# gerbenvoshol/kmer-cnt

Hardware: AMD Instinct MI355X
Metric: Mbases/sec (+ k-mers/sec) on 150 bp FASTQ, k=21 (higher is better)
Workload: dtype u8

## Files before the change

### include/vafc.h

```cpp
#ifndef VAFC_H
#define VAFC_H

#include <stddef.h>
#include <stdint.h>

#ifdef __cplusplus
extern "C" {
#endif

#define VAFC_VERSION_MAJOR 0
#define VAFC_VERSION_MINOR 1

enum {
	VC_OK = 0,
	VC_EINVAL = -1,
	VC_ENOMEM = -2,
	VC_EHIP = -3,
	VC_ENODEV = -4,
	VC_EIO = -5,
	VC_ETOOMANY = -6,
	VC_EFULL = -7
};

typedef struct vc_ctx vc_ctx;
typedef struct vc_patterns vc_patterns;


int vc_patterns_load(const char *path, vc_patterns **out);
void vc_patterns_free(vc_patterns *db);
int vc_patterns_count(const vc_patterns *db);

int vc_patterns_keys(const vc_patterns *db, int k, uint64_t **keys, uint32_t **vals,
                     size_t *n_keys, int *n_collisions);

int vc_write_vaf(const vc_patterns *db, const uint32_t *counts, const char *path);

int vc_pattern_fields(const vc_patterns *db, int i, const char **chr, int *start,
                      const char **rsid, char *ref, char *alt,
                      const char **ref_kmer, const char **alt_kmer);

void vc_free(void *p);


int vc_create(vc_ctx **out, int k, const uint64_t *keys, const uint32_t *vals,
              size_t n_keys, uint32_t n_patterns, int device);
void vc_destroy(vc_ctx *ctx);

int vc_count_block(vc_ctx *ctx, const uint8_t *seq, size_t seq_bytes,
                   const uint64_t *offs, const uint32_t *lens, uint64_t n_reads);

#define VC_STREAM_CTX ((void *)(intptr_t)-1)

int vc_count_device(vc_ctx *ctx, const uint8_t *d_seq, size_t seq_bytes,
                    const uint64_t *d_offs, const uint32_t *d_lens, uint64_t n_reads,
                    void *stream);

int vc_finish(vc_ctx *ctx, uint32_t *counts, uint64_t *kmers_extracted);

int vc_reset(vc_ctx *ctx);

void *vc_device_counts(vc_ctx *ctx);
int vc_bind_outputs(vc_ctx *ctx, void *d_counts, void *d_tally);
void *vc_device_tally(vc_ctx *ctx);
void *vc_stream(vc_ctx *ctx);

int vc_set_timing(vc_ctx *ctx, int enable);
int vc_kernel_ms(vc_ctx *ctx, float *ms);

int vc_table_info(const vc_ctx *ctx, uint64_t *n_keys, uint64_t *slots, uint64_t *filter_bytes);


#define VC_MAX_SHARDS 64

int vc_create_multi(vc_ctx **out, int k, const uint64_t *keys, const uint32_t *vals, size_t n_keys,
                    uint32_t n_patterns, const int *devices, int n_devices);
int vc_shard_count(const vc_ctx *ctx);
int vc_shard_info(const vc_ctx *ctx, int i, int *device, uint64_t *batches);


typedef struct {
	uint64_t bases;
	uint64_t seqs;
	uint64_t blocks;
	double seconds;
} vc_file_stats;

int vc_count_file(vc_ctx *ctx, const char *path, int block_bases, int n_threads,
                  vc_file_stats *st);

typedef struct {
	uint64_t first;
	uint64_t next;
	uint64_t errs;
	uint32_t stopped;
	uint32_t whole;
} vc_range_info;
int vc_count_file_range(vc_ctx *ctx, const char *path, uint64_t begin, uint64_t end, int block_bases,
                        int n_threads, vc_file_stats *st, vc_range_info *ri);
int vc_scan_file_range(const char *path, int k, int block_bases, int n_threads, uint64_t piece_bytes,
                       uint64_t begin, uint64_t end, vc_file_stats *st, vc_range_info *ri, uint8_t *seq_out,
                       size_t seq_cap, uint32_t *lens_out, size_t lens_cap);

uint64_t vc_ingest_profile(double *prof);

#define VC_INGEST_PROFILE_FIELDS 17
uint64_t vc_ingest_profile_ex(double *prof, int n);

int vc_reserve_file_ingest(vc_ctx *ctx, int n_threads);

int vc_scan_file(const char *path, int k, int block_bases, vc_file_stats *st,
                 uint8_t *seq_out, size_t seq_cap, uint32_t *lens_out, size_t lens_cap);

int vc_scan_file_parallel(const char *path, int k, int block_bases, int n_threads, uint64_t piece_bytes,
                          vc_file_stats *st, uint8_t *seq_out, size_t seq_cap, uint32_t *lens_out,
                          size_t lens_cap);

int64_t vc_gz_inflate_parallel(const char *path, int n_threads, uint64_t chunk_bytes, uint8_t *out,
                               uint64_t cap, uint64_t *stats6);
int64_t vc_gz_inflate_zlib(const char *path, uint8_t *out, uint64_t cap);
uint32_t vc_gz_crc32(uint32_t crc, const uint8_t *p, uint64_t n);
uint32_t vc_gz_crc32_combine(uint32_t crc1, uint32_t crc2, uint64_t len2);

typedef struct {
	uint64_t start_bit;
	uint64_t end_bit;
	uint64_t text_len;
	uint32_t ok;
	uint32_t ended;
} vc_gz_share_info;
int vc_gz_share_scan(const char *path, uint64_t begin, uint64_t end, int n_threads, uint64_t chunk_bytes,
                     vc_gz_share_info *out, uint16_t *window_sym);

typedef struct {
	uint32_t events;
	uint32_t head_crc;
	uint64_t head_len;
	uint32_t head_expect_crc;
	uint32_t head_expect_isize;
	uint32_t tail_crc;
	uint64_t tail_len;
	uint32_t crc_error;
	uint32_t complete;
} vc_gz_share_crc;
int vc_count_gz_share(vc_ctx *ctx, const char *path, int first_share, uint64_t start_bit, const uint8_t *window,
                      uint64_t text_len, int block_bases, int n_threads, vc_file_stats *st, vc_range_info *ri,
                      vc_gz_share_crc *crc);
int vc_scan_gz_share(const char *path, int k, int first_share, uint64_t start_bit, const uint8_t *window,
                     uint64_t text_len, int block_bases, int n_threads, vc_file_stats *st, vc_range_info *ri,
                     vc_gz_share_crc *crc, uint8_t *seq_out, size_t seq_cap, uint32_t *lens_out, size_t lens_cap);

typedef struct vc_gz_share vc_gz_share;
int vc_gz_share_open(vc_ctx *ctx, const char *path, uint64_t begin, uint64_t end, int n_threads,
                     uint64_t chunk_bytes, uint64_t hold_bytes, vc_gz_share_info *out, uint16_t *window_sym,
                     vc_gz_share **held);
int vc_count_gz_share_held(vc_ctx *ctx, vc_gz_share *held, int first_share, const uint8_t *window, uint64_t text_len,
                           int block_bases, int n_threads, vc_file_stats *st, vc_range_info *ri, vc_gz_share_crc *crc);
int vc_scan_gz_share_held(vc_gz_share *held, int k, int first_share, const uint8_t *window, uint64_t text_len,
                          int block_bases, int n_threads, vc_file_stats *st, vc_range_info *ri, vc_gz_share_crc *crc,
                          uint8_t *seq_out, size_t seq_cap, uint32_t *lens_out, size_t lens_cap);
void vc_gz_share_close(vc_gz_share *held);

int64_t vc_scan_records(const char *path, int32_t *rets, int64_t cap);


typedef struct vc_fasta vc_fasta;
int vc_fasta_load(const char *path, vc_fasta **out);
int vc_fasta_count(const vc_fasta *fa);
const char *vc_fasta_name(const vc_fasta *fa, int i);
const uint8_t *vc_fasta_seq(const vc_fasta *fa, int i, uint32_t *len);
int vc_fasta_data(const vc_fasta *fa, const uint8_t **seq, size_t *bytes, const uint64_t **offs,
                  const uint32_t **lens);
void vc_fasta_free(vc_fasta *fa);


int vc_kc_create(vc_ctx **out, int k, uint64_t table_slots, int device);
int vc_kc_set_partition(vc_ctx *ctx, uint32_t n_parts, uint32_t part);
uint64_t vc_kc_slots(vc_ctx *ctx);
int vc_kc_histogram(vc_ctx *ctx, uint64_t *hist, uint64_t *distinct, uint64_t *kmers);
int vc_kc_histogram2(vc_ctx *ctx, uint64_t *hist, uint32_t n_bins, uint64_t min_count, uint64_t *distinct,
                     uint64_t *kmers);

int vc_kc_track_first(vc_ctx *ctx, int on);
int vc_yak_bloom_select(vc_ctx *ctx, int pre, int bf_shift, int n_hash);

int vc_set_nt4_decode(vc_ctx *ctx, int on);

int vc_count_candidates(int k, const uint8_t *seq, size_t seq_bytes, const uint64_t *offs,
                        const uint32_t *lens, uint64_t n_seqs, const uint64_t *keys, size_t n_keys,
                        uint32_t *counts, int device);


typedef struct vc_vafset vc_vafset;
int vc_vafset_create(vc_vafset **out);
void vc_vafset_free(vc_vafset *s);
int vc_vafset_add(vc_vafset *s, const char *path);
int vc_vafset_add_many(vc_vafset *s, const char *const *paths, int n, int n_threads, int *n_added,
                       uint8_t *truncated);
int vc_vafset_add_arrays(vc_vafset *s, const char *name, const double *vaf, const int32_t *depth, int n);
int vc_vafset_count(const vc_vafset *s);
const char *vc_vafset_name(const vc_vafset *s, int i);
int vc_vafset_snps(const vc_vafset *s, int i);
int vc_corr_matrix(const vc_vafset *s, int min_snps, int min_depth, double *corr, int device, float *kernel_ms);
int vc_corr_matrix_raw(const double *vaf, const int32_t *depth, const int32_t *n_snps, int n_samples,
                       size_t stride, int min_snps, int min_depth, double *corr, int device, float *kernel_ms);
int vc_corr_write(const vc_vafset *s, const double *corr, const char *path);
int vc_corr_tree(const vc_vafset *s, const double *corr, const char *path);


typedef struct vc_ed vc_ed;

int vc_ed_create(vc_ed **out, const vc_patterns *db, int max_edit, int device);
int vc_ed_create_raw(vc_ed **out, const uint8_t *queries, const uint32_t *q_offs, const uint32_t *q_lens,
                     size_t n_queries, int max_edit, int device);
void vc_ed_destroy(vc_ed *ed);
int vc_ed_count_block(vc_ed *ed, const uint8_t *seq, size_t seq_bytes, const uint64_t *offs, const uint32_t *lens,
                      uint64_t n_reads);
int vc_ed_count_device(vc_ed *ed, const uint8_t *d_seq, size_t seq_bytes, const uint64_t *d_offs,
                       const uint32_t *d_lens, uint64_t n_reads, void *stream);
int vc_ed_finish(vc_ed *ed, uint32_t *counts);
int vc_ed_reset(vc_ed *ed);
int vc_ed_set_counts(vc_ed *ed, const uint32_t *counts);
int vc_ed_set_max_ranges(vc_ed *ed, uint32_t max_ranges);
int vc_ed_shape(const vc_ed *ed, int width, uint32_t *n_groups, int *waves, int *lds_masks);
int vc_ed_kernel_ms(vc_ed *ed, float *ms);
int vc_ed_count_file(vc_ed *ed, const char *path, int n_threads, vc_file_stats *st);



typedef struct {
	int32_t tid, pos;
	uint32_t flag, n_cigar, l_seq;
	uint32_t reserved;
	uint64_t off;
} vc_bam_rec;

typedef struct vc_bam vc_bam;
typedef struct vc_bam_file vc_bam_file;

enum { VC_BAM_BGZF = 0, VC_BAM_SAM = 1, VC_BAM_CRAM = 2, VC_BAM_RAW = 3, VC_BAM_GZIP = 4, VC_BAM_BGZF_OTHER = 5 };
int vc_bam_probe(const char *path, int *kind);
const char *vc_bam_kind_name(int kind);

int vc_bam_read_file(const char *path, int n_threads, vc_bam_file **out);
int vc_bam_read_header(const char *path, vc_bam_file **out);
int vc_bam_file_refs(const vc_bam_file *f);
const char *vc_bam_file_ref_name(const vc_bam_file *f, int i);
uint64_t vc_bam_file_records(const vc_bam_file *f, const vc_bam_rec **recs, const uint8_t **data, uint64_t *data_bytes);
void vc_bam_file_free(vc_bam_file *f);
int vc_bam_index_usable(const char *path, char *buf, size_t buf_len);
int vc_bam_build_regions(const vc_patterns *db, int32_t *first_row, int32_t *ends);

int vc_bam_create(vc_bam **out, const vc_patterns *db, const char *const *ref_names, int n_refs, int device);
void vc_bam_destroy(vc_bam *b);
int vc_bam_set_regions(vc_bam *b, const int32_t *tid, const int32_t *start, const int32_t *end, size_t n);
int vc_bam_count_block(vc_bam *b, const vc_bam_rec *recs, uint64_t n_recs, const uint8_t *data, size_t data_bytes);
int vc_bam_count_device(vc_bam *b, const vc_bam_rec *d_recs, uint64_t n_recs, const uint8_t *d_data,
                        size_t data_bytes, void *stream);
int vc_bam_finish(vc_bam *b, uint32_t *counts);
int vc_bam_reset(vc_bam *b);
int vc_bam_set_counts(vc_bam *b, const uint32_t *counts);
int vc_bam_set_long_threshold(vc_bam *b, uint32_t ops);
int vc_bam_kernel_ms(vc_bam *b, float *ms);
int vc_bam_count_file(vc_bam *b, const char *path, int n_threads, vc_file_stats *st);



typedef struct vc_vcf vc_vcf;
typedef struct vc_vcf_header vc_vcf_header;

#define VC_VCF_TILE_BYTES 4096

typedef struct {
	uint64_t off;
	int32_t row;
	uint32_t reserved;
} vc_vcf_hit;

enum { VC_VCF_PLAIN = 0, VC_VCF_GZIP = 1, VC_VCF_BGZF = 2, VC_VCF_BCF = 3, VC_VCF_OTHER = 4 };
int vc_vcf_probe(const char *path, int *kind);
const char *vc_vcf_kind_name(int kind);

#define VC_VCF_MORE 1
#define VC_VCF_ABORTED 2
int vc_vcf_header_parse(const uint8_t *text, size_t len, int final, vc_vcf_header **out, size_t *body_off);
int vc_vcf_header_samples(const vc_vcf_header *h);
int vc_vcf_header_type(const vc_vcf_header *h, const char *tag);
void vc_vcf_header_free(vc_vcf_header *h);

enum { VC_VCF_SKIP = 0, VC_VCF_SET = 1, VC_VCF_END = 2, VC_VCF_ABORT = 3 };
typedef struct {
	int32_t verdict;
	int32_t head_ok;
	int64_t pos;
	uint32_t chrom_len;
	int32_t n_allele;
	uint32_t ref_len, alt_len;
	uint8_t ref, alt;
	uint8_t reserved[2];
	uint32_t ref_count, alt_count;
} vc_vcf_verdict;
int vc_vcf_eval_line(const vc_vcf_header *h, const uint8_t *line, size_t len, int sample_idx, int min_depth,
                     vc_vcf_verdict *out);

int vc_vcf_create(vc_vcf **out, const vc_patterns *db, int device);
int vc_vcf_create_raw(vc_vcf **out, const char *const *chr, const int32_t *start, const char *ref, const char *alt,
                      size_t n, size_t table_slots, int device);
void vc_vcf_destroy(vc_vcf *v);
int vc_vcf_scan_block(vc_vcf *v, const uint8_t *text, size_t len, uint64_t file_off, int final, size_t *consumed);
int vc_vcf_scan_device(vc_vcf *v, const uint8_t *d_text, size_t len, uint64_t file_off, int final, void *stream);
int vc_vcf_hits(vc_vcf *v, const vc_vcf_hit **hits, size_t *n_hits, size_t *consumed);
int vc_vcf_set_max_hits(vc_vcf *v, size_t max_hits);
int vc_vcf_set_block_bytes(vc_vcf *v, size_t bytes);
int vc_vcf_kernel_ms(vc_vcf *v, float *ms);
int vc_vcf_count_file(vc_vcf *v, const char *path, int sample_idx, int min_depth, int n_threads, uint32_t *counts,
                      vc_file_stats *st);


int vc_synth_reads(uint8_t *d_seq, uint64_t *d_offs, uint32_t *d_lens, uint64_t first,
                   uint64_t n_reads, uint32_t read_len, uint64_t seed, double f_snp,
                   const uint8_t *d_windows, const uint8_t *d_dosage, uint32_t n_snp,
                   void *stream);

int vc_debug_decode(const uint8_t *d_seq, size_t seq_bytes, const uint64_t *d_offs,
                    const uint32_t *d_lens, uint64_t n_reads, uint8_t *d_codes, void *stream);

const char *vc_strerror(int err);
int vc_version(void);
const char *vc_build_id(void);

#ifdef __cplusplus
}
#endif
#endif
```

### kmer-cnt_amd/csrc/vafc_host.cpp

```cpp
#include <hip/hip_runtime.h>
#include <rccl/rccl.h>

#include <ctype.h>
#include <dlfcn.h>
#include <sched.h>
#include <fcntl.h>
#include <math.h>
#include <sys/mman.h>
#include <sys/stat.h>
#include <unistd.h>
#include <stdio.h>
#include <stdlib.h>
#include <string.h>

#include <mutex>
#include <vector>

#include "vafc.h"
#include "vafc_affinity.h"
#include "vafc_common.h"
#include "vafc_fastq.h"
#include "vafc_gzip.h"
#include "vafc_ingest.h"
#include "vafc_internal.h"
// ... 380 lines not shown
	if (!c) return VC_EINVAL;
	if (!c->kc)
		for (int i = 0; i < n_shards(c); ++i) {
			vc_ctx *sh = shard_at(c, i);
			uint32_t f = 0;
			HIPCK(hipSetDevice(sh->dev));
			HIPCK(hipStreamSynchronize(sh->st));
			HIPCK(hipMemcpy(&f, sh->d_flags, sizeof f, hipMemcpyDeviceToHost));
			if (f & 1u) {
				fprintf(stderr, "[E::vafc] more reads longer than %d bases than the long-read list holds "
				        "(overlapping device reads?): counts incomplete\n", VC_LONG_READ);
				return VC_EINVAL;
			}
		}
	if (!c->rep.empty()) {
		int rc = reduce_shards(c);
		if (rc != VC_OK) return rc;
	}
	HIPCK(hipSetDevice(c->dev));
	HIPCK(hipStreamSynchronize(c->st));
	c->stage.settle();
	if (c->kc) {
		unsigned long long st[4];
		HIPCK(hipMemcpy(st, c->kc->d_stats, sizeof st, hipMemcpyDeviceToHost));
		if (kmers) *kmers = st[0];
		if (st[3]) {
			fprintf(stderr, "[E::vafc] more reads longer than %d bases than the long-read list holds "
			        "(overlapping reads?): counts incomplete\n", KC_LONG);
			return VC_EINVAL;
		}
		return VC_OK;
	}
	if (counts)
		HIPCK(hipMemcpy(counts, c->d_counts, 2 * (size_t)c->n_patterns * sizeof(uint32_t),
		                hipMemcpyDeviceToHost));
	if (kmers) {
		unsigned long long t = 0;
		HIPCK(hipMemcpy(&t, c->d_tally, sizeof(t), hipMemcpyDeviceToHost));
		*kmers = t;
	}
	return VC_OK;
}

extern "C" int vc_reset(vc_ctx *c)
{
	if (!c) return VC_EINVAL;
	HIPCK(hipSetDevice(c->dev));
	if (c->kc) {
		Kc &K = *c->kc;
		HIPCK(hipMemsetAsync(K.d_table, 0, K.slots * 16, c->st));
		HIPCK(hipMemsetAsync(K.d_stats, 0, 4 * sizeof(unsigned long long), c->st));
		if (K.track_first) HIPCK(hipMemsetAsync(K.d_first, 0xFF, K.slots * 8, c->st));
		K.read_base = 0;
		K.lookup_only = false;
		return VC_OK;
	}
	HIPCK(hipMemsetAsync(c->d_counts, 0, 2 * (size_t)c->n_patterns * sizeof(uint32_t), c->st));
	HIPCK(hipMemsetAsync(c->d_tally, 0, sizeof(unsigned long long), c->st));
	HIPCK(hipMemsetAsync(c->d_flags, 0, sizeof(uint32_t), c->st));
	for (vc_ctx *r : c->rep) {
		int rc = vc_reset(r);
		if (rc != VC_OK) return rc;
	}
	return VC_OK;
}

extern "C" void *vc_device_counts(vc_ctx *c) { return c ? (void *)c->d_counts : nullptr; }
extern "C" int vc_bind_outputs(vc_ctx *c, void *d_counts, void *d_tally)
{
	if (!c) return VC_EINVAL;
	c->d_counts = d_counts ? (uint32_t *)d_counts : c->own_counts;
	c->d_tally = d_tally ? (unsigned long long *)d_tally : c->own_tally;
	return VC_OK;
}

extern "C" void *vc_device_tally(vc_ctx *c) { return c ? (void *)c->d_tally : nullptr; }
extern "C" void *vc_stream(vc_ctx *c) { return c ? (void *)c->st : nullptr; }

extern "C" int vc_set_timing(vc_ctx *c, int enable)
{
	if (!c) return VC_EINVAL;
	c->timing = enable != 0;
	c->timer.clear();
	return VC_OK;
}

extern "C" int vc_kernel_ms(vc_ctx *c, float *ms) { return c ? c->timer.ms(ms) : VC_EINVAL; }

extern "C" int vc_table_info(const vc_ctx *c, uint64_t *n_keys, uint64_t *slots, uint64_t *filter_bytes)
{
	if (!c) return VC_EINVAL;
	if (n_keys) *n_keys = c->n_keys;
	if (slots) *slots = (uint64_t)1 << c->tbits;
	if (filter_bytes) *filter_bytes = (uint64_t)4 * c->fwords;
	return VC_OK;
}


namespace {

struct RcclApi {
	bool tried = false, ok = false;
	decltype(&ncclCommInitAll) comm_init_all = nullptr;
	decltype(&ncclCommDestroy) comm_destroy = nullptr;
	decltype(&ncclReduce) reduce = nullptr;
	decltype(&ncclGroupStart) group_start = nullptr;
	decltype(&ncclGroupEnd) group_end = nullptr;
	decltype(&ncclGetErrorString) error_string = nullptr;
};
RcclApi g_rccl;
std::mutex g_rccl_mu;

const RcclApi *rccl()
{
	std::lock_guard<std::mutex> lk(g_rccl_mu);
	if (g_rccl.tried) return g_rccl.ok ? &g_rccl : nullptr;
	g_rccl.tried = true;
	const char *env = getenv("VAFC_RCCL_LIB");
	void *h = dlopen(env && *env ? env : "librccl.so.1", RTLD_NOW | RTLD_GLOBAL);
	if (!h && !(env && *env)) h = dlopen("librccl.so", RTLD_NOW | RTLD_GLOBAL);
	if (!h) {
		fprintf(stderr, "[E::vafc] cannot load RCCL: %s\n", dlerror());
		return nullptr;
	}
	RcclApi &R = g_rccl;
	R.comm_init_all = (decltype(R.comm_init_all))dlsym(h, "ncclCommInitAll");
	R.comm_destroy = (decltype(R.comm_destroy))dlsym(h, "ncclCommDestroy");
	R.reduce = (decltype(R.reduce))dlsym(h, "ncclReduce");
	R.group_start = (decltype(R.group_start))dlsym(h, "ncclGroupStart");
	R.group_end = (decltype(R.group_end))dlsym(h, "ncclGroupEnd");
	R.error_string = (decltype(R.error_string))dlsym(h, "ncclGetErrorString");
	R.ok = R.comm_init_all && R.comm_destroy && R.reduce && R.group_start && R.group_end && R.error_string;
	if (!R.ok) fprintf(stderr, "[E::vafc] RCCL lacks the symbols vafc needs\n");
	return R.ok ? &R : nullptr;
}

}

#define NCCK(R, call)                                                                               \
	do {                                                                                            \
		ncclResult_t e_ = (call);                                                                   \
		if (e_ != ncclSuccess) {                                                                    \
			fprintf(stderr, "[E::vafc] %s failed: %s (%s:%d)\n", #call, (R)->error_string(e_),      \
			        __FILE__, __LINE__);                                                            \
			return VC_EHIP;                                                                         \
		}                                                                                           \
	} while (0)

static void rccl_comms_destroy(vc_ctx *c)
{
	if (c->comms.empty()) return;
	const RcclApi *R = rccl();
	if (R)
		for (ncclComm_t m : c->comms) (void)R->comm_destroy(m);
	c->comms.clear();
	c->comm_shard.clear();
}

extern "C" int vc_create_multi(vc_ctx **out, int k, const uint64_t *keys, const uint32_t *vals, size_t n_keys,
                               uint32_t n_patterns, const int *devices, int n_devices)
{
	if (!out || !devices || n_devices < 1 || n_devices > VC_MAX_SHARDS) return VC_EINVAL;
	*out = nullptr;
	int n_distinct = 0;
	for (int i = 0; i < n_devices; ++i) {
		bool seen = false;
		for (int j = 0; j < i; ++j) seen = seen || devices[j] == devices[i];
		n_distinct += seen ? 0 : 1;
	}
	if (n_distinct > 1 && !rccl()) return VC_EHIP;
	vc_ctx *c = nullptr;
	int rc = vc_create(&c, k, keys, vals, n_keys, n_patterns, devices[0]);
	if (rc != VC_OK) return rc;
	c->lead.assign(1, 0);
	for (int i = 1; i < n_devices; ++i) {
		vc_ctx *r = nullptr;
		if ((rc = vc_create(&r, k, keys, vals, n_keys, n_patterns, devices[i])) != VC_OK) {
			vc_destroy(c);
			return rc;
		}
		c->rep.push_back(r);
		int l = i;
		for (int j = 0; j < i; ++j)
			if (devices[j] == devices[i]) {
				l = j;
				break;
			}
		c->lead.push_back(l);
	}
	if (n_distinct > 1) {
		const RcclApi *R = rccl();
		std::vector<int> devs;
		for (int i = 0; i < n_devices; ++i)
			if (c->lead[(size_t)i] == i) {
				devs.push_back(devices[i]);
				c->comm_shard.push_back(i);
			}
		c->comms.assign(devs.size(), nullptr);
		const ncclResult_t e = R->comm_init_all(c->comms.data(), (int)devs.size(), devs.data());
		if (e != ncclSuccess) {
			fprintf(stderr, "[E::vafc] ncclCommInitAll over %d devices failed: %s\n", (int)devs.size(),
			        R->error_string(e));
			c->comms.clear();
			vc_destroy(c);
			return VC_EHIP;
		}
	}
	*out = c;
	return VC_OK;
}

static int reduce_shards(vc_ctx *c)
{
	const int N = n_shards(c);
	const size_t n = 2 * (size_t)c->n_patterns;
	for (int i = 0; i < N; ++i) {
		vc_ctx *sh = shard_at(c, i);
		HIPCK(hipSetDevice(sh->dev));
		HIPCK(hipStreamSynchronize(sh->st));
	}
	for (int i = 0; i < N; ++i) {
		const int l = c->lead[(size_t)i];
		if (l == i) continue;
		vc_ctx *L = shard_at(c, l), *S = shard_at(c, i);
		HIPCK(hipSetDevice(L->dev));
		HIPCK(vc_launch_shard_add(L->d_counts, S->d_counts, n, L->d_tally, S->d_tally, L->st));
	}
	if (c->comms.size() <= 1) {
		HIPCK(hipSetDevice(c->dev));
		HIPCK(hipStreamSynchronize(c->st));
		return VC_OK;
	}
	const RcclApi *R = rccl();
	if (!R) return VC_EHIP;
	NCCK(R, R->group_start());
	ncclResult_t first = ncclSuccess;
	for (size_t j = 0; j < c->comms.size() && first == ncclSuccess; ++j) {
		vc_ctx *L = shard_at(c, c->comm_shard[j]);
		(void)hipSetDevice(L->dev);
		if (n) first = R->reduce(L->d_counts, L->d_counts, n, ncclUint32, ncclSum, 0, c->comms[j], L->st);
		if (first == ncclSuccess)
			first = R->reduce(L->d_tally, L->d_tally, 1, ncclUint64, ncclSum, 0, c->comms[j], L->st);
	}
	const ncclResult_t ge = R->group_end();
	if (first == ncclSuccess) first = ge;
	if (first != ncclSuccess) {
		fprintf(stderr, "[E::vafc] RCCL reduce of the shard counts failed: %s\n", R->error_string(first));
		return VC_EHIP;
	}
	for (size_t j = 1; j < c->comms.size(); ++j) {
		vc_ctx *L = shard_at(c, c->comm_shard[j]);
		HIPCK(hipSetDevice(L->dev));
		HIPCK(hipMemsetAsync(L->d_counts, 0, n * sizeof(uint32_t), L->st));
		HIPCK(hipMemsetAsync(L->d_tally, 0, sizeof(unsigned long long), L->st));
	}
	for (size_t j = 0; j < c->comms.size(); ++j) {
		vc_ctx *L = shard_at(c, c->comm_shard[j]);
		HIPCK(hipSetDevice(L->dev));
		HIPCK(hipStreamSynchronize(L->st));
	}
	return VC_OK;
}

extern "C" int vc_shard_count(const vc_ctx *c) { return c ? n_shards(c) : 0; }

extern "C" int vc_shard_info(const vc_ctx *c, int i, int *device, uint64_t *batches)
{
	if (!c || i < 0 || i >= n_shards(c)) return VC_EINVAL;
	const vc_ctx *sh = shard_at(const_cast<vc_ctx *>(c), i);
	if (device) *device = sh->dev;
	if (batches) *batches = sh->batches;
	return VC_OK;
}


#ifndef VC_BATCH_BYTES
#define VC_BATCH_BYTES ((size_t)64 << 20)
#endif


#ifndef VC_PIECE_BYTES
#define VC_PIECE_BYTES ((uint64_t)16 << 20)
#endif
#ifndef VC_PIECE_BYTES_WARM
#define VC_PIECE_BYTES_WARM ((uint64_t)32 << 20)
#endif

static int ingest_slot_alloc(VcSlot &s, uint64_t piece);
static size_t ingest_slot_bytes(uint64_t piece);

namespace {

class DeviceSink : public VcIngestSink {
public:
	DeviceSink(vc_ctx *c, uint64_t piece) : c_(c), n_(n_shards(c)), piece_(piece) {}
	int acquire(int slot, VcSlotBuf *b) override
	{
		vc_ctx *sh;
		VcSlot &s = at(slot, &sh);
		HIPCK(hipSetDevice(sh->dev));
		int rc = vc_slot_wait(s);
		if (rc != VC_OK) return rc;
		if (!s.h_seq || s.cap_bytes < ingest_slot_bytes(piece_)) rc = ingest_slot_alloc(s, piece_);
		if (rc == VC_OK) fill(s, b);
		return rc;
	}
	int grow(int slot, VcSlotBuf *b, size_t bytes, size_t reads, size_t used_bytes, size_t used_reads) override
	{
		vc_ctx *sh;
		VcSlot &s = at(slot, &sh);
		HIPCK(hipSetDevice(sh->dev));
		const int rc = vc_slot_realloc(s, bytes, reads, used_bytes, used_reads);
		if (rc == VC_OK) fill(s, b);
		return rc;
	}
	int submit(int slot, const VcSlotBuf &, uint64_t n, uint64_t bytes) override
	{
		vc_ctx *sh;
		VcSlot &s = at(slot, &sh);
		HIPCK(hipSetDevice(sh->dev));
		if (!sh->cst) HIPCK(hipStreamCreateWithFlags(&sh->cst, hipStreamNonBlocking));
		if (!s.copied) HIPCK(hipEventCreateWithFlags(&s.copied, hipEventDisableTiming));
		HIPCK(hipMemcpyAsync(s.d_seq, s.h_seq, bytes, hipMemcpyHostToDevice, sh->cst));
		HIPCK(hipMemcpyAsync(s.d_offs, s.h_offs, n * sizeof(uint64_t), hipMemcpyHostToDevice, sh->cst));
		HIPCK(hipMemcpyAsync(s.d_lens, s.h_lens, n * sizeof(uint32_t), hipMemcpyHostToDevice, sh->cst));
		HIPCK(hipEventRecord(s.copied, sh->cst));
		HIPCK(hipStreamWaitEvent(sh->st, s.copied, 0));
		int rc = launch(sh, s.d_seq, bytes, s.d_offs, s.d_lens, n, sh->st, any_long(s.h_lens, n));
		if (rc != VC_OK) return rc;
		HIPCK(hipEventRecord(s.done, sh->st));
		s.pending = true;
		++sh->batches;
		return VC_OK;
	}

private:
	vc_ctx *c_;
	int n_;
	uint64_t piece_;
	VcSlot &at(int slot, vc_ctx **sh)
	{
		*sh = shard_at(c_, slot % n_);
		return (*sh)->islot[(size_t)(slot / n_)];
	}
	static void fill(const VcSlot &s, VcSlotBuf *b)
	{
		b->seq = s.h_seq;
		b->offs = s.h_offs;
		b->lens = s.h_lens;
		b->cap_bytes = s.cap_bytes;
		b->cap_reads = s.cap_reads;
	}
};

}

#ifndef VC_PARALLEL_MIN_BYTES
#define VC_PARALLEL_MIN_BYTES ((uint64_t)32 << 20)
#endif

static int clamp_threads(int n) { return n < 1 ? 1 : (n > 64 ? 64 : n); }

static int reserve_ingest_slots(vc_ctx *c, size_t slots, bool alloc);

static int reserve_ingest(vc_ctx *c, int threads, bool alloc)
{
	const int N = n_shards(c);
	const char *e = getenv("VAFC_INGEST_SLOTS");
	const int want = e && atoi(e) > threads ? atoi(e) : (threads < 2 ? threads + 2 : 2 * threads);
	const int slots = (want + N - 1) / N * N;
	for (int i = 0; i < N; ++i) {
		vc_ctx *sh = shard_at(c, i);
		HIPCK(hipSetDevice(sh->dev));
		int rc = reserve_ingest_slots(sh, (size_t)(slots / N), alloc);
		if (rc != VC_OK) return rc;
	}
	return slots;
}

static size_t ingest_slot_bytes(uint64_t piece) { return (size_t)piece / 2 + ((size_t)256 << 10); }

static int slot_alloc_mapped(VcSlot &s, size_t bytes, size_t reads)
{
	const size_t huge = (size_t)2 << 20;
	const size_t ob = (bytes + 63) / 64 * 64, lb = ob + reads * sizeof(uint64_t);
	const size_t need = lb + reads * sizeof(uint32_t);
	const size_t len = (need + huge - 1) / huge * huge;
	void *m = mmap(nullptr, len + huge, PROT_READ | PROT_WRITE, MAP_PRIVATE | MAP_ANONYMOUS, -1, 0);
	if (m == MAP_FAILED) return VC_ENOMEM;
	uint8_t *a = (uint8_t *)(((uintptr_t)m + huge - 1) / huge * huge);
	if (a > (uint8_t *)m) munmap(m, (size_t)(a - (uint8_t *)m));
	const size_t tail = (size_t)((uint8_t *)m + len + huge - (a + len));
	if (tail) munmap(a + len, tail);
	madvise(a, len, MADV_HUGEPAGE);
	for (size_t i = 0; i < len; i += 4096) a[i] = 0;
	if (hipHostRegister(a, len, hipHostRegisterDefault) != hipSuccess) {
		(void)hipGetLastError();
		munmap(a, len);
		return VC_EHIP;
	}
	uint8_t *d = nullptr;
	if (hipMalloc(&d, need) != hipSuccess) {
		(void)hipGetLastError();
		(void)hipHostUnregister(a);
		munmap(a, len);
		return VC_EHIP;
	}
	s.map = a;
	s.map_len = len;
	s.h_seq = a;
	s.h_offs = (uint64_t *)(a + ob);
	s.h_lens = (uint32_t *)(a + lb);
	s.d_seq = d;
	s.d_offs = (uint64_t *)(d + ob);
	s.d_lens = (uint32_t *)(d + lb);
	s.d_one = true;
	s.cap_bytes = bytes;
	s.cap_reads = reads;
	return VC_OK;
}

static int ingest_slot_alloc(VcSlot &s, uint64_t piece)
{
	static const bool use_malloc = getenv("VAFC_PIN") && !strcmp(getenv("VAFC_PIN"), "malloc");
	const size_t bytes = ingest_slot_bytes(piece), reads = (size_t)piece / 256 + 4096;
	if (use_malloc) return vc_slot_reserve(s, bytes, reads);
	if (bytes <= s.cap_bytes && reads <= s.cap_reads) return VC_OK;
	const int rc = vc_slot_wait(s);
	if (rc != VC_OK) return rc;
	vc_slot_free(s);
	return slot_alloc_mapped(s, bytes + bytes / 4 + 4096, reads + reads / 4 + 1024);
}

static int reserve_ingest_slots(vc_ctx *c, size_t slots, bool alloc)
{
	if (c->islot.size() < slots) {
		HIPCK(hipStreamSynchronize(c->st));
		const size_t old = c->islot.size();
		c->islot.resize(slots);
		for (size_t i = old; i < slots; ++i)
			HIPCK(hipEventCreateWithFlags(&c->islot[i].done, hipEventDisableTiming));
	}
	for (size_t i = 0; alloc && i < slots; ++i) {
		VcSlot &s = c->islot[i];
		if (s.h_seq) continue;
		int rc = ingest_slot_alloc(s, VC_PIECE_BYTES);
		if (rc != VC_OK) return rc;
	}
	return VC_OK;
}

extern "C" int vc_reserve_file_ingest(vc_ctx *c, int n_threads)
{
	if (!c) return VC_EINVAL;
	const int rc = reserve_ingest(c, clamp_threads(n_threads), true);
	return rc < 0 ? rc : VC_OK;
}

static int count_file_parallel(vc_ctx *c, int fd, uint64_t size, int block_bases, int n_threads,
                               vc_file_stats &st, VcTextRange *range = nullptr)
{
	const int threads = clamp_threads(n_threads);
	const int slots = reserve_ingest(c, threads, false);
	if (slots < 0) return slots;
	const uint64_t piece = vc_ingest_piece(c->ingest_warm ? VC_PIECE_BYTES_WARM : VC_PIECE_BYTES);
	DeviceSink sink(c, piece);
	const int rc = vc_ingest_plain(fd, size, c->k, block_bases, threads, slots, piece, sink, st, range);
	if (rc == VC_OK) c->ingest_warm = true;
	return rc;
}

static int count_file_gzip(vc_ctx *c, VcGzParallel *g, int block_bases, int n_threads, vc_file_stats &st)
{
	const int parsers = vc_gz_parse_threads(clamp_threads(n_threads));
	const int slots = reserve_ingest(c, parsers, false);
	if (slots < 0) return slots;
	const uint64_t piece = vc_ingest_piece(VC_PIECE_BYTES);
	DeviceSink sink(c, piece);
	return vc_ingest_gzip(g, c->k, block_bases, parsers, slots, piece, (uint64_t)(slots + 2) * piece * 2, sink, st);
}

static int sync_shards(vc_ctx *c)
{
	for (int i = 0; i < n_shards(c); ++i) {
		vc_ctx *sh = shard_at(c, i);
		HIPCK(hipSetDevice(sh->dev));
		HIPCK(hipStreamSynchronize(sh->st));
	}
	return hipSetDevice(c->dev) == hipSuccess ? VC_OK : VC_EHIP;
}

static VcCpuSet gpu_cpus(vc_ctx *c, int threads)
{
	if (c->cpus_threads == threads) return c->cpus;
	VcCpuSet out;
	const char *ne = getenv("VAFC_NUMA");
	cpu_set_t mask;
	CPU_ZERO(&out.set);
	if (!(ne && !strcmp(ne, "0")) && sched_getaffinity(0, sizeof mask, &mask) == 0) {
		bool any_node = false, bad = false;
		for (int i = 0; i < n_shards(c) && !bad; ++i) {
			char bus[64] = {0}, path[256], buf[4096];
			if (hipDeviceGetPCIBusId(bus, (int)sizeof bus, shard_at(c, i)->dev) != hipSuccess) {
				(void)hipGetLastError();
				bad = true;
				break;
			}
			for (char *q = bus; *q; ++q) *q = (char)tolower((unsigned char)*q);
			snprintf(path, sizeof path, "/sys/bus/pci/devices/%s/numa_node", bus);
			FILE *f = fopen(path, "r");
			int node = -1;
			if (!f || fscanf(f, "%d", &node) != 1) node = -1;
			if (f) fclose(f);
			if (node < 0) {
				bad = true;
				break;
			}
			snprintf(path, sizeof path, "/sys/devices/system/node/node%d/cpulist", node);
			f = fopen(path, "r");
			size_t n = f ? fread(buf, 1, sizeof buf - 1, f) : 0;
			if (f) fclose(f);
			buf[n] = 0;
			for (char *q = buf; *q;) {
				char *e;
				const long a = strtol(q, &e, 10);
				if (e == q) break;
				long b = a;
				if (*e == '-') b = strtol(e + 1, &e, 10);
				for (long x = a; x <= b && x < CPU_SETSIZE; ++x) CPU_SET((int)x, &out.set);
				any_node = true;
				q = *e == ',' ? e + 1 : e;
				if (*e != ',') break;
			}
		}
		if (!bad && any_node) {
			CPU_AND(&out.set, &out.set, &mask);
			const int have = CPU_COUNT(&out.set);
			out.on = have >= threads && have < CPU_COUNT(&mask);
		}
	}
	c->cpus = out;
	c->cpus_threads = threads;
	return out;
}

static VcCpuSet reader_cpus(vc_ctx *c, int threads, bool gz)
{
	return gpu_cpus(c, gz ? vc_gz_inflate_threads(threads) + vc_gz_parse_threads(threads) + 2 : threads);
}

namespace {

struct FilePass {
	vc_ctx *c;
	vc_file_stats *out;
	vc_file_stats st = {0, 0, 0, 0.0};
	double t0 = vc_now();

	FilePass(vc_ctx *ctx, vc_file_stats *o) : c(ctx), out(o) {}
	int finish(int rc)
	{
		if (rc == VC_OK && c) rc = sync_shards(c);
		st.seconds = vc_now() - t0;
		if (out) *out = st;
		return rc;
	}
};

struct FileKind {
	int fd = -1;
	bool regular = false, gzip = false;
	uint64_t size = 0;
};

bool classify(const char *path, FileKind *f)
{
	struct stat sb;
	if (stat(path, &sb) != 0) return false;
	if (!S_ISREG(sb.st_mode)) return true;
	if ((f->fd = open(path, O_RDONLY)) < 0) return false;
	uint8_t magic[2] = {0, 0};
	f->regular = fstat(f->fd, &sb) == 0 && S_ISREG(sb.st_mode);
	f->gzip = f->regular && pread(f->fd, magic, 2, 0) == 2 && magic[0] == 0x1f && magic[1] == 0x8b;
	f->size = f->regular ? (uint64_t)sb.st_size : 0;
	return true;
}

}

extern "C" int vc_count_file(vc_ctx *c, const char *path, int block_bases, int n_threads,
                             vc_file_stats *st)
{
	if (!c || !path) return VC_EINVAL;
	HIPCK(hipSetDevice(c->dev));
	FilePass fp(c, st);
	FileKind f;
	if (!classify(path, &f)) return fp.finish(VC_EIO);
	const int t = clamp_threads(n_threads);
	VcAffinityScope placement(reader_cpus(c, t, f.gzip));
	const char *me = getenv("VAFC_INGEST_MIN");
	const uint64_t min_bytes = me ? (uint64_t)atoll(me) : VC_PARALLEL_MIN_BYTES;
	if (f.regular && !f.gzip && f.size >= min_bytes && f.size > 0) {
		const int rc = count_file_parallel(c, f.fd, f.size, block_bases, n_threads, fp.st);
		close(f.fd);
		return fp.finish(rc);
	}
	if (f.fd >= 0) close(f.fd);
	if (f.gzip) {
		VcGzParallel *g = vc_gzp_open(path, vc_gz_inflate_threads(t), vc_gz_chunk());
		if (g) {
			const int rc = count_file_gzip(c, g, block_bases, n_threads, fp.st);
			vc_gzp_close(g);
			return fp.finish(rc);
		}
	}
	VcFastqReader rd;
	if (!rd.open_parallel(path, t)) return fp.finish(VC_EIO);
	const size_t limit = vc_batch_bytes(VC_BATCH_BYTES);
	VcBatchWriter bw(limit, limit / 64, [c]() -> vc_ctx * {
		vc_ctx *sh = next_shard(c);
		return hipSetDevice(sh->dev) == hipSuccess ? sh : nullptr;
	});
	int rc = vc_block_loop(rd, c->k, block_bases, [&bw](const char *s, size_t l) { return bw.add(s, l); }, fp.st);
	if (rc == VC_OK) rc = bw.flush();
	return fp.finish(rc);
}

extern "C" int vc_count_file_range(vc_ctx *c, const char *path, uint64_t begin, uint64_t end, int block_bases,
                                   int n_threads, vc_file_stats *st, vc_range_info *ri)
{
	if (!c || !path || !ri || end <= begin) return VC_EINVAL;
	*ri = vc_range_info{UINT64_MAX, UINT64_MAX, 0, 0, 1};
	HIPCK(hipSetDevice(c->dev));
	FilePass fp(c, st);
	FileKind f;
	if (!classify(path, &f)) return fp.finish(VC_EIO);
	if (!f.regular || f.gzip) {
		if (f.fd >= 0) close(f.fd);
		int rc = VC_OK;
		if (begin == 0) {
			rc = vc_count_file(c, path, block_bases, n_threads, &fp.st);
			if (rc == VC_OK) *ri = vc_range_info{0, UINT64_MAX, 0, 1, 1};
		}
		return fp.finish(rc);
	}
	VcTextRange R;
	R.begin = begin;
	R.end = end;
	int rc;
	{
		VcAffinityScope placement(reader_cpus(c, clamp_threads(n_threads), false));
		rc = count_file_parallel(c, f.fd, f.size, block_bases, n_threads, fp.st, &R);
	}
	close(f.fd);
	*ri = vc_range_info{R.first, R.next, R.errs, R.stopped ? 1u : 0u, 0u};
	return fp.finish(rc);
}

static int count_gz_share_g(vc_ctx *c, VcGzParallel *g, int fmt, int parsers, int first_share,
                            const uint8_t *window, uint64_t text_len, int block_bases, vc_file_stats &local,
                            vc_range_info *ri, vc_gz_share_crc *crc)
{
	int rc = reserve_ingest(c, parsers, false);
	VcTextRange R;
	const size_t np = first_share ? 0 : 1;
	if (rc >= 0) {
		const int slots = rc;
		const uint64_t piece = vc_ingest_piece(VC_PIECE_BYTES);
		DeviceSink sink(c, piece);
		R.begin = np;
		R.end = np + text_len;
		R.format = fmt;
		rc = vc_ingest_gzip_share(g, first_share ? nullptr : window + 32767, np, c->k, block_bases, parsers, slots,
		                          piece, (uint64_t)(slots + 2) * piece * 2, sink, local, &R);
	}
	VcGzShareCrc sc;
	vc_gzp_share_crc(g, &sc);
	vc_gzp_close(g);
	*ri = vc_range_info{R.first == UINT64_MAX ? UINT64_MAX : R.first - np,
	                    R.next == UINT64_MAX ? UINT64_MAX : R.next - np - text_len, R.errs, R.stopped ? 1u : 0u, 0u};
	*crc = vc_gz_share_crc{sc.events, sc.head_crc, sc.head_len, sc.head_expect_crc, sc.head_expect_isize,
	                       sc.tail_crc, sc.tail_len, sc.crc_error, sc.complete};
	return rc;
}

extern "C" int vc_count_gz_share(vc_ctx *c, const char *path, int first_share, uint64_t start_bit,
                                 const uint8_t *window, uint64_t text_len, int block_bases, int n_threads,
                                 vc_file_stats *st, vc_range_info *ri, vc_gz_share_crc *crc)
{
	if (!c || !path || !ri || !crc || text_len == 0 || (!first_share && !window)) return VC_EINVAL;
	*ri = vc_range_info{UINT64_MAX, UINT64_MAX, 0, 0, 0};
	memset(crc, 0, sizeof *crc);
	HIPCK(hipSetDevice(c->dev));
	FilePass fp(c, st);
	const int fmt = vc_gz_text_format(path);
	if (fmt < 0) return fp.finish(VC_EINVAL);
	const int t = clamp_threads(n_threads);
	VcAffinityScope placement(reader_cpus(c, t, true));
	VcGzParallel *g = vc_gzp_open_share(path, vc_gz_inflate_threads(t), vc_gz_chunk(), first_share != 0, start_bit,
	                                    window, text_len);
	if (!g) return fp.finish(VC_EIO);
	return fp.finish(count_gz_share_g(c, g, fmt, vc_gz_parse_threads(t), first_share, window, text_len, block_bases,
	                                  fp.st, ri, crc));
}

extern "C" int vc_gz_share_open(vc_ctx *c, const char *path, uint64_t begin, uint64_t end, int n_threads,
                                uint64_t chunk_bytes, uint64_t hold_bytes, vc_gz_share_info *out,
                                uint16_t *window_sym, vc_gz_share **held)
{
	if (!path || !out || !held || end <= begin) return VC_EINVAL;
	*held = nullptr;
	const int t = n_threads < 1 ? 1 : n_threads;
	VcCpuSet none;
	CPU_ZERO(&none.set);
	if (c) HIPCK(hipSetDevice(c->dev));
	VcAffinityScope placement(c ? reader_cpus(c, clamp_threads(t), true) : none);
	VcGzShare sh;
	VcGzParallel *g = nullptr;
	if (!vc_gzp_scan_share_hold(path, t, chunk_bytes, begin, end, hold_bytes, &sh, window_sym, &g)) return VC_EIO;
// ... 263 lines not shown
```

### kmer-cnt_amd/csrc/vafc_ingest.cpp

```cpp
#include "vafc_ingest.h"
#include "vafc_affinity.h"

#include <errno.h>
#include <stdio.h>
#include <stdlib.h>
#include <string.h>
#include <time.h>
#include <sys/mman.h>
#include <immintrin.h>
#include <unistd.h>

#include <atomic>
#include <condition_variable>
#include <deque>
#include <mutex>
#include <thread>
#include <vector>

#include "vafc_fastq.h"
#include "vafc_gzip.h"

namespace {

struct Piece {
	uint64_t j = 0;
	uint64_t a = 0, b = 0;
	int64_t start = -1;
	uint64_t end = 0;
	bool eof = false;
	uint64_t n = 0, bytes = 0;
	std::vector<uint64_t> errs;
	VcSlotBuf buf;
	int rc = VC_OK;
	bool ready = false;
};

double ing_clock(clockid_t id)
{
	struct timespec ts;
	clock_gettime(id, &ts);
	return ts.tv_sec + ts.tv_nsec * 1e-9;
}

struct IoTally {
	double read_s = 0;
	uint64_t read_bytes = 0;
};
thread_local IoTally io_tally;

ssize_t pread_full(int fd, uint8_t *p, size_t n, uint64_t off)
{
	size_t got = 0;
	while (got < n) {
		ssize_t r = pread(fd, p + got, n - got, (off_t)(off + got));
		if (r < 0 && errno == EINTR) continue;
		if (r <= 0) break;
		got += (size_t)r;
	}
	return (ssize_t)got;
}

int slot_copy_mode()
{
	const char *e = getenv("VAFC_SLOT_COPY");
	return e && e[0] >= '0' && e[0] <= '2' ? e[0] - '0' : 2;
}

class SlotCopier {
public:
	explicit SlotCopier(int mode) : mode_(mode) {}
	void bind(uint8_t *dst) { dst_ = dst; }
	void add(const char *src, size_t len, uint64_t at, bool in_window)
	{
		if (mode_ == 0) {
			memcpy(dst_ + at, src, len);
			return;
		}
		if (!in_window || len > kStage / 2) {
			flush();
			const double t0 = ing_clock(CLOCK_MONOTONIC);
			memcpy(dst_ + at, src, len);
			secs += ing_clock(CLOCK_MONOTONIC) - t0;
			bytes += len;
			return;
		}
		if (!ents_.empty() && (pend_ + len > kStage || at != d1_)) flush();
		if (ents_.empty()) d0_ = d1_ = at;
		ents_.push_back({(const uint8_t *)src, (uint32_t)len});
		d1_ += len;
		pend_ += len;
		if (pend_ >= kStage / 2) flush();
	}
	void flush()
	{
		if (ents_.empty()) return;
		const double t0 = ing_clock(CLOCK_MONOTONIC);
		uint8_t *d = dst_ + d0_;
		if (mode_ == 1) {
			for (const Ent &e : ents_) {
				memcpy(d, e.src, e.len);
				d += e.len;
			}
		} else {
			uint8_t *s = stage_;
			for (const Ent &e : ents_) {
				memcpy(s, e.src, e.len);
				s += e.len;
			}
			stream(d, stage_, pend_);
		}
		secs += ing_clock(CLOCK_MONOTONIC) - t0;
		bytes += pend_;
		ents_.clear();
		pend_ = 0;
	}
	void finish()
	{
		flush();
		if (mode_ == 2) _mm_sfence();
	}
	static void refill_hook(void *self) { ((SlotCopier *)self)->flush(); }
	double secs = 0;
	uint64_t bytes = 0;

private:
	struct Ent {
		const uint8_t *src;
		uint32_t len;
	};
	static constexpr size_t kStage = (size_t)32 << 10;
	int mode_;
	uint8_t *dst_ = nullptr;
	std::vector<Ent> ents_;
	uint64_t d0_ = 0, d1_ = 0;
	size_t pend_ = 0;
	alignas(64) uint8_t stage_[kStage];

	__attribute__((target("avx2"))) static void stream_avx2(uint8_t *d, const uint8_t *s, size_t n)
	{
		const size_t head = (size_t)((64 - ((uintptr_t)d & 63)) & 63);
		if (n < head + 64) {
			memcpy(d, s, n);
			return;
		}
		memcpy(d, s, head);
		d += head;
		s += head;
		n -= head;
		for (; n >= 64; n -= 64, d += 64, s += 64) {
			const __m256i a = _mm256_loadu_si256((const __m256i *)s);
			const __m256i b = _mm256_loadu_si256((const __m256i *)(s + 32));
			_mm256_stream_si256((__m256i *)d, a);
			_mm256_stream_si256((__m256i *)(d + 32), b);
		}
		memcpy(d, s, n);
	}
	static void stream(uint8_t *d, const uint8_t *s, size_t n)
	{
		static const bool avx2 = __builtin_cpu_supports("avx2");
		if (avx2) stream_avx2(d, s, n);
		else memcpy(d, s, n);
	}
};

class FdSource : public VcIngestSource {
public:
	FdSource(int fd, uint64_t size) : fd_(fd), size_(size)
	{
		const char *e = getenv("VAFC_MMAP");
		if (size_ > 0 && e && e[0] == '1') {
			void *m = mmap(nullptr, (size_t)size_, PROT_READ, MAP_SHARED, fd_, 0);
			if (m != MAP_FAILED) map_ = (const uint8_t *)m;
		}
	}
	~FdSource() override
	{
		if (map_) munmap((void *)map_, (size_t)size_);
	}
	int64_t read(uint8_t *p, size_t n, uint64_t off) override
	{
		const double t0 = ing_clock(CLOCK_MONOTONIC);
		int64_t got;
		if (!map_) {
			got = pread_full(fd_, p, n, off);
		} else if (off >= size_) {
			got = 0;
		} else {
			got = (int64_t)(size_ - off < n ? (size_t)(size_ - off) : n);
			memcpy(p, map_ + off, (size_t)got);
		}
		io_tally.read_s += ing_clock(CLOCK_MONOTONIC) - t0;
		io_tally.read_bytes += got > 0 ? (uint64_t)got : 0;
		return got;
	}
	const uint8_t *view(uint64_t off, uint64_t *avail) override
	{
		*avail = map_ && off < size_ ? size_ - off : 0;
		return map_ && off <= size_ ? map_ + off : nullptr;
	}
	bool longer_than(uint64_t off) override { return size_ > off; }

private:
	int fd_;
	uint64_t size_;
	const uint8_t *map_ = nullptr;
};

class GzSource : public VcIngestSource {
public:
	GzSource(VcGzParallel *g, uint64_t window, const uint8_t *prefix = nullptr, size_t np = 0) : g_(g), window_(window)
	{
		if (np) {
			Block *b = new Block;
			uint8_t *c = (uint8_t *)malloc(np);
			memcpy(c, prefix, np);
			b->p = c;
			b->len = np;
			blocks_.push_back(b);
			end_ = np;
		}
		pump_ = std::thread([this, cpus = vc_affinity_get()] {
			vc_affinity_bind(cpus);
			pump();
		});
	}
	~GzSource() override
	{
		abort();
		pump_.join();
		for (Block *b : blocks_) {
			drop(b);
		}
	}
	int64_t read(uint8_t *p, size_t n, uint64_t off) override
	{
		std::vector<std::pair<const uint8_t *, size_t>> seg;
		size_t got = 0;
		{
			std::unique_lock<std::mutex> lk(mu_);
			wait_for(lk, off + n);
			if (end_ <= off) return 0;
			got = (size_t)(end_ - off < n ? end_ - off : n);
			size_t need = got;
			uint64_t pos = off;
			for (Block *b : blocks_) {
				if (!need) break;
				if (b->off + b->len <= pos) continue;
				const size_t from = (size_t)(pos - b->off);
				const size_t take = b->len - from < need ? b->len - from : need;
				seg.emplace_back(b->p + from, take);
				pos += take;
				need -= take;
			}
		}
		size_t at = 0;
		for (auto &sg : seg) {
			memcpy(p + at, sg.first, sg.second);
			at += sg.second;
		}
		return (int64_t)got;
	}
	bool longer_than(uint64_t off) override
	{
		std::unique_lock<std::mutex> lk(mu_);
		wait_for(lk, off + 1);
		return end_ > off;
	}
	void release(uint64_t off) override
	{
		std::lock_guard<std::mutex> lk(mu_);
		if (off <= rel_) return;
		rel_ = off;
		while (blocks_.size() > 1 && blocks_.front()->off + blocks_.front()->len <= rel_) {
			drop(blocks_.front());
			blocks_.pop_front();
		}
		room_.notify_all();
	}
	void abort() override
	{
		std::lock_guard<std::mutex> lk(mu_);
		aborted_ = true;
		data_.notify_all();
		room_.notify_all();
	}

private:
	struct Block {
		uint64_t off = 0;
		size_t len = 0;
		const uint8_t *p = nullptr;
		void *hold = nullptr;
	};
	VcGzParallel *g_;
	uint64_t window_;
	std::thread pump_;
	std::mutex mu_;
	std::condition_variable data_, room_;
	std::deque<Block *> blocks_;
	uint64_t end_ = 0, rel_ = 0;
	int waiting_ = 0;
	bool eof_ = false, aborted_ = false;

	void wait_for(std::unique_lock<std::mutex> &lk, uint64_t want)
	{
		while (end_ < want && !eof_ && !aborted_) {
			++waiting_;
			room_.notify_all();
			data_.wait(lk);
			--waiting_;
		}
	}
	const bool copy_ = getenv("VAFC_GZ_COPY") != nullptr;
	void drop(Block *b)
	{
		if (b->hold) vc_gzp_release(g_, b->hold);
		else free((void *)b->p);
		delete b;
	}
	void pump()
	{
		for (;;) {
			{
				std::unique_lock<std::mutex> lk(mu_);
				room_.wait(lk, [&] { return aborted_ || end_ - rel_ < window_ || waiting_ > 0; });
				if (aborted_) break;
			}
			const uint8_t *q = nullptr;
			void *h = nullptr;
			const int64_t n = copy_ ? vc_gzp_span(g_, &q, (size_t)8 << 20)
			                        : vc_gzp_span_hold(g_, &q, (size_t)64 << 20, &h);
			if (n <= 0) break;
			Block *nb = new Block;
			if (copy_) {
				uint8_t *c = (uint8_t *)malloc((size_t)n);
				if (!c) {
					delete nb;
					break;
				}
				memcpy(c, q, (size_t)n);
				q = c;
			}
			nb->p = q;
			nb->len = (size_t)n;
			nb->hold = h;
			std::lock_guard<std::mutex> lk(mu_);
			nb->off = end_;
			blocks_.push_back(nb);
			end_ += (uint64_t)n;
			data_.notify_all();
		}
		std::lock_guard<std::mutex> lk(mu_);
		eof_ = true;
		data_.notify_all();
	}
};

const uint8_t *find_nl(const uint8_t *p, const uint8_t *e)
{
	return p < e ? (const uint8_t *)memchr(p, '\n', (size_t)(e - p)) : nullptr;
}

int64_t guess_in(const uint8_t *s, size_t n, uint64_t from, bool at_eof, bool fasta)
{
	const uint8_t *e = s + n;
	for (const uint8_t *p = s + 1; p < e; ++p) {
		if (p[-1] != '\n') {
			p = find_nl(p, e);
			if (!p) return -1;
			continue;
		}
		if (fasta) {
			if (*p == '>' || *p == '@') return (int64_t)(from + (uint64_t)(p - s));
			continue;
		}
		if (*p != '@') continue;
		const uint8_t *n1 = find_nl(p, e);
		const uint8_t *n2 = n1 ? find_nl(n1 + 1, e) : nullptr;
		if (!n2) return -1;
		if (n2 + 1 >= e) {
			if (!at_eof) return -1;
			continue;
		}
		if (n2[1] != '+') continue;
		const uint8_t *n3 = find_nl(n2 + 1, e);
		if (!n3) return -1;
		const uint8_t *n4 = find_nl(n3 + 1, e);
		const uint8_t *qe = n4 ? n4 : (at_eof ? e : nullptr);
		if (!qe) return -1;
		if (qe - (n3 + 1) != n2 - (n1 + 1)) continue;
		if (n4 && n4 + 1 < e && n4[1] != '@') continue;
		if (n4 && n4 + 1 >= e && !at_eof) return -1;
		return (int64_t)(from + (uint64_t)(p - s));
	}
	return -1;
}

int64_t guess_record(VcTextSource &src, uint64_t a, bool fasta, std::vector<uint8_t> &tmp)
{
	const uint64_t from = a - 1;
	const size_t cap = (size_t)1 << 20;
	uint64_t avail = 0;
	const uint8_t *v = src.view(from, &avail);
	if (v) {
		const size_t got = (size_t)(avail < cap ? avail : cap);
		return got < 2 ? -1 : guess_in(v, got, from, got < cap, fasta);
	}
	tmp.resize(cap);
	size_t have = 0;
	for (size_t want = (size_t)16 << 10;; want = want * 8 < cap ? want * 8 : cap) {
		const int64_t got = src.read(tmp.data() + have, want - have, from + have);
		have += got > 0 ? (size_t)got : 0;
		const bool at_eof = have < want;
		if (have < 2) return -1;
		const int64_t g = guess_in(tmp.data(), have, from, at_eof, fasta);
		if (g >= 0 || at_eof || want == cap) return g;
	}
}

int parse_piece(VcTextSource &src, uint64_t start, int k, int slot, VcIngestSink &sink, VcFastqReader &rd,
                Piece &P, SlotCopier &cp)
{
	P.start = (int64_t)start;
	P.n = P.bytes = 0;
	P.errs.clear();
	P.eof = false;
	P.end = start;
	uint64_t avail = 0;
	const uint8_t *v = src.view(start, &avail);
	const char *we = getenv("VAFC_READER_WINDOW");
	const size_t win = we && atoll(we) > 0 ? (size_t)atoll(we) : (size_t)1 << 20;
	if (!(v ? rd.open_view(v, avail, start) : rd.open_src(&src, start, win))) return VC_ENOMEM;
	cp.bind(P.buf.seq);
	rd.on_refill(SlotCopier::refill_hook, &cp);
	struct Unhook {
		VcFastqReader &r;
		SlotCopier &c;
		~Unhook()
		{
			c.finish();
			r.on_refill(nullptr, nullptr);
		}
	} unhook{rd, cp};
	size_t used = 0;
	for (;;) {
		const int64_t h = rd.peek_header();
		if (h < 0) {
			P.eof = true;
			P.end = UINT64_MAX;
			break;
		}
		if ((uint64_t)h >= P.b) {
			P.end = (uint64_t)h;
			break;
		}
		const int ret = rd.next();
		if (ret == -1) {
			P.eof = true;
			P.end = UINT64_MAX;
			break;
		}
		if (ret == -2) {
			P.errs.push_back(P.n);
			continue;
		}
		if (ret < k) continue;
		const size_t len = (size_t)ret;
		if (used + len > P.buf.cap_bytes || P.n + 1 > P.buf.cap_reads) {
			size_t nb = P.buf.cap_bytes, nr = P.buf.cap_reads;
			while (used + len > nb) nb = nb * 2 + len;
			while (P.n + 1 > nr) nr = nr * 2 + 1024;
			cp.flush();
			int rc = sink.grow(slot, &P.buf, nb, nr, used, (size_t)P.n);
			if (rc != VC_OK) return rc;
			cp.bind(P.buf.seq);
		}
		cp.add(rd.seq(), len, used, rd.seq_in_window());
		P.buf.offs[P.n] = used;
		P.buf.lens[P.n] = (uint32_t)len;
		used += len;
		P.bytes += len;
		++P.n;
	}
	return VC_OK;
}

struct BlockState {
	int64_t sum = 0;
	int empty = 0;
	bool stopped = false;
};

uint64_t replay_blocks(const Piece &P, int block_bases, BlockState &S, vc_file_stats &st)
{
	uint64_t keep = 0;
	size_t e = 0;
	auto end_block = [&]() {
		if (S.sum == 0) {
			if (++S.empty >= 3) S.stopped = true;
		} else {
			++st.blocks;
		}
		S.sum = 0;
	};
	for (uint64_t i = 0; i <= P.n && !S.stopped; ++i) {
		while (e < P.errs.size() && P.errs[e] == i && !S.stopped) {
			end_block();
			++e;
		}
		if (S.stopped || i == P.n) break;
		const uint32_t len = P.buf.lens[i];
		S.sum += len;
		st.bases += len;
		st.seqs += 1;
		keep = i + 1;
		if (S.sum >= block_bases) {
			++st.blocks;
			S.sum = 0;
		}
	}
	if (P.eof && !S.stopped) {
		end_block();
		S.stopped = true;
	}
	return keep;
}

}

thread_local VcIngestProfile vc_ingest_last;

static double ing_now()
{
	struct timespec ts;
	clock_gettime(CLOCK_MONOTONIC, &ts);
	return ts.tv_sec + ts.tv_nsec * 1e-9;
}

int vc_ingest_text(VcIngestSource &src, int k, int block_bases, int threads, int slots, uint64_t piece_bytes,
                   VcIngestSink &sink, vc_file_stats &st, VcTextRange *range)
{
	const bool prof_print = getenv("VAFC_INGEST_PROFILE") != nullptr;
	const int copy_mode = slot_copy_mode();
	vc_ingest_last = VcIngestProfile();
	double t_wait = 0, t_submit = 0, t_reparse = 0;
	std::atomic<uint64_t> t_parse_us{0}, t_slotwait_us{0}, t_acquire_us{0};
	const double t_begin = ing_now();
	if (threads < 1 || slots < threads + 1 || piece_bytes < 2) return VC_EINVAL;
	const uint64_t r0 = range ? range->begin : 0, r1 = range ? range->end : UINT64_MAX;
	if (range) {
		if (r1 <= r0) return VC_EINVAL;
		range->first = r0 == 0 ? 0 : UINT64_MAX;
		range->next = UINT64_MAX;
		range->errs = 0;
		range->stopped = false;
	}
	if (!src.longer_than(r0)) {
		if (range) range->first = UINT64_MAX;
		return VC_OK;
	}
	if (!src.longer_than(0)) return VC_OK;
	bool fasta = false;
	if (range && range->format >= 0) {
		fasta = range->format == 1;
	} else {
		VcFastqReader rd;
		if (!rd.open_src(&src, 0, (size_t)1 << 16)) return VC_ENOMEM;
		const int64_t h = rd.peek_header();
		if (h < 0) {
			if (range) range->first = UINT64_MAX;
			return VC_OK;
		}
		uint8_t c = 0;
		if (src.read(&c, 1, (uint64_t)h) == 1) fasta = c == '>';
	}
	std::vector<Piece> pcs((size_t)slots);
	std::mutex mu;
	std::condition_variable cv;
	uint64_t released = 0;
	uint64_t n_pieces = UINT64_MAX;
	bool abort = false;
	std::atomic<uint64_t> next{0};

	const VcCpuSet cpus = vc_affinity_get();
	std::atomic<uint64_t> w_read_ns{0}, w_read_bytes{0}, w_copy_ns{0}, w_copy_bytes{0}, w_guess_ns{0};
	std::atomic<uint64_t> w_cpu_ns{0}, w_wall_ns{0};
	auto worker_loop = [&](VcFastqReader &rd, std::vector<uint8_t> &tmp, SlotCopier &cp) {
		for (;;) {
			const uint64_t j = next.fetch_add(1);
			const double w0 = ing_now();
			{
				std::unique_lock<std::mutex> lk(mu);
				cv.wait(lk, [&] { return abort || released + (uint64_t)slots > j; });
				if (abort || j >= n_pieces) return;
			}
			const uint64_t pa = r0 + j * piece_bytes;
			if (pa >= r1 || !src.longer_than(pa)) {
				std::lock_guard<std::mutex> lk(mu);
				if (j < n_pieces) n_pieces = j;
				cv.notify_all();
				return;
			}
			const double w1 = ing_now();
			const int slot = (int)(j % (uint64_t)slots);
			Piece &P = pcs[(size_t)slot];
			P.j = j;
			P.a = pa;
			P.b = r1 - pa > piece_bytes ? pa + piece_bytes : r1;
			int rc = sink.acquire(slot, &P.buf);
			t_acquire_us += (uint64_t)((ing_now() - w1) * 1e6);
			if (rc == VC_OK) {
				const double g0 = ing_now();
				const int64_t g = P.a == 0 ? 0 : guess_record(src, P.a, fasta, tmp);
				w_guess_ns += (uint64_t)((ing_now() - g0) * 1e9);
				if (g >= 0) rc = parse_piece(src, (uint64_t)g, k, slot, sink, rd, P, cp);
				else P.start = -1;
			}
			{
				const double w2 = ing_now();
				t_slotwait_us += (uint64_t)((w1 - w0) * 1e6);
				t_parse_us += (uint64_t)((w2 - w1) * 1e6);
			}
			std::lock_guard<std::mutex> lk(mu);
			P.rc = rc;
			P.ready = true;
			cv.notify_all();
		}
	};
	auto worker = [&]() {
		vc_affinity_bind(cpus);
		const double c0 = ing_clock(CLOCK_THREAD_CPUTIME_ID), t0 = ing_now();
		io_tally = IoTally();
		VcFastqReader rd;
		std::vector<uint8_t> tmp;
		SlotCopier cp(copy_mode);
		worker_loop(rd, tmp, cp);
		w_read_ns += (uint64_t)(io_tally.read_s * 1e9);
		w_read_bytes += io_tally.read_bytes;
		w_copy_ns += (uint64_t)(cp.secs * 1e9);
		w_copy_bytes += cp.bytes;
		w_cpu_ns += (uint64_t)((ing_clock(CLOCK_THREAD_CPUTIME_ID) - c0) * 1e9);
		w_wall_ns += (uint64_t)((ing_now() - t0) * 1e9);
	};
	const double main_cpu0 = ing_clock(CLOCK_THREAD_CPUTIME_ID);
	std::vector<std::thread> pool;
	for (int t = 0; t < threads; ++t) pool.emplace_back(worker);

	int rc = VC_OK;
	BlockState S;
	uint64_t expect = 0;
	uint64_t np = 0;
	VcFastqReader rd;
	SlotCopier mcp(copy_mode);
	for (uint64_t j = 0;; ++j) {
		const int slot = (int)(j % (uint64_t)slots);
		Piece &P = pcs[(size_t)slot];
		const double m0 = ing_now();
		{
			std::unique_lock<std::mutex> lk(mu);
			cv.wait(lk, [&] { return (P.ready && P.j == j) || n_pieces <= j; });
			if (!(P.ready && P.j == j)) break;
		}
		np = j + 1;
		t_wait += ing_now() - m0;
		if (rc == VC_OK) rc = P.rc;
		if (j == 0 && r0 > 0) {
			if (P.start < 0) {
				src.release(P.a);
				std::lock_guard<std::mutex> lk(mu);
				P.ready = false;
				released = 1;
				abort = true;
				cv.notify_all();
				break;
			}
			expect = (uint64_t)P.start;
			if (range) range->first = expect;
		}
		if (rc == VC_OK && !S.stopped && P.b > expect) {
			if (P.start < 0 || (uint64_t)P.start != expect) {
				const double r0 = ing_now();
				rc = parse_piece(src, expect, k, slot, sink, rd, P, mcp);
				t_reparse += ing_now() - r0;
			}
			if (rc == VC_OK) {
				expect = P.end;
				if (range) range->errs += P.errs.size();
				const uint64_t keep = replay_blocks(P, block_bases, S, st);
				if (keep) {
					const uint64_t bytes = (uint64_t)P.buf.offs[keep - 1] + P.buf.lens[keep - 1];
					const double s0 = ing_now();
					rc = sink.submit(slot, P.buf, keep, bytes);
					t_submit += ing_now() - s0;
				}
			}
		}
		const uint64_t nxt = r0 + (j + 1) * piece_bytes - 1;
		src.release(expect < nxt ? expect : nxt);
		const bool done = rc != VC_OK || S.stopped;
		{
			std::lock_guard<std::mutex> lk(mu);
			P.ready = false;
			released = j + 1;
			if (done) abort = true;
			cv.notify_all();
		}
		if (done) break;
	}
	src.abort();
	for (auto &t : pool) t.join();
	{
		VcIngestProfile &L = vc_ingest_last;
		L.total = ing_now() - t_begin;
		L.main_wait = t_wait;
		L.submit = t_submit;
		L.reparse = t_reparse;
		L.parse = (t_parse_us.load() - t_acquire_us.load()) * 1e-6;
		L.slot_wait = t_slotwait_us.load() * 1e-6;
		L.acquire = t_acquire_us.load() * 1e-6;
		L.pieces = np;
		L.threads = threads;
		L.read_s = w_read_ns.load() * 1e-9;
		L.read_bytes = w_read_bytes.load();
		L.copy_s = w_copy_ns.load() * 1e-9;
		L.copy_bytes = w_copy_bytes.load();
		L.guess_s = w_guess_ns.load() * 1e-9;
		L.worker_cpu = w_cpu_ns.load() * 1e-9;
		L.worker_wall = w_wall_ns.load() * 1e-9;
		L.main_cpu = ing_clock(CLOCK_THREAD_CPUTIME_ID) - main_cpu0;
		L.copy_mode = copy_mode;
	}
	if (prof_print) {
		const VcIngestProfile &L = vc_ingest_last;
		fprintf(stderr, "[ingest] %llu pieces, %d threads: total %.6f s; main: wait %.6f submit %.6f reparse %.6f "
		        "cpu %.6f; workers: parse %.6f slot-wait %.6f acquire %.6f (thread-seconds); parse split: read %.6f "
		        "(%.2f GB) copy %.6f (%.2f GB, mode %d) guess %.6f; workers cpu %.6f of wall %.6f\n",
		        (unsigned long long)np, threads, L.total, t_wait, t_submit, t_reparse, L.main_cpu, L.parse,
		        L.slot_wait, L.acquire, L.read_s, L.read_bytes / 1e9, L.copy_s, L.copy_bytes / 1e9, L.copy_mode,
		        L.guess_s, L.worker_cpu, L.worker_wall);
	}
	if (range) {
		range->stopped = S.stopped;
		range->next = S.stopped ? UINT64_MAX : expect;
		if (range->first == UINT64_MAX) range->next = UINT64_MAX;
		return rc;
	}
	if (rc == VC_OK && !S.stopped) {
		rc = VC_EINVAL;
	}
	return rc;
}

int vc_ingest_plain(int fd, uint64_t size, int k, int block_bases, int threads, int slots,
                    uint64_t piece_bytes, VcIngestSink &sink, vc_file_stats &st, VcTextRange *range)
{
	FdSource src(fd, size);
	return vc_ingest_text(src, k, block_bases, threads, slots, piece_bytes, sink, st, range);
}

int vc_ingest_gzip(VcGzParallel *g, int k, int block_bases, int threads, int slots, uint64_t piece_bytes,
                   uint64_t window_bytes, VcIngestSink &sink, vc_file_stats &st)
{
	GzSource src(g, window_bytes);
	return vc_ingest_text(src, k, block_bases, threads, slots, piece_bytes, sink, st);
}

int vc_ingest_gzip_share(VcGzParallel *g, const uint8_t *prefix, size_t np, int k, int block_bases, int threads,
                         int slots, uint64_t piece_bytes, uint64_t window_bytes, VcIngestSink &sink, vc_file_stats &st,
                         VcTextRange *range)
{
	GzSource src(g, window_bytes, prefix, np);
	return vc_ingest_text(src, k, block_bases, threads, slots, piece_bytes, sink, st, range);
}

int vc_gz_text_format(const char *path)
{
	gzFile f = gzopen(path, "r");
	if (!f) return -1;
	uint8_t buf[1 << 16];
	int fmt = -1;
	for (size_t seen = 0; fmt < 0 && seen < ((size_t)1 << 20);) {
		const int n = gzread(f, buf, sizeof buf);
		if (n <= 0) break;
		for (int i = 0; i < n; ++i)
			if (buf[i] == '>' || buf[i] == '@') {
				fmt = buf[i] == '>' ? 1 : 0;
				break;
			}
		seen += (size_t)n;
	}
	gzclose(f);
	return fmt;
}


#include <fcntl.h>
#include <stdlib.h>
#include <sys/stat.h>
#include <time.h>

namespace {

class HostSink : public VcIngestSink {
public:
	HostSink(int slots, uint64_t piece, uint8_t *seq_out, size_t seq_cap, uint32_t *lens_out, size_t lens_cap)
		: bufs_((size_t)slots), piece_(piece), seq_out_(seq_out), seq_cap_(seq_cap), lens_out_(lens_out),
		  lens_cap_(lens_cap) {}
	~HostSink() override
	{
		for (auto &b : bufs_) {
			free(b.seq);
			free(b.offs);
			free(b.lens);
		}
	}
	int acquire(int slot, VcSlotBuf *b) override
	{
		VcSlotBuf &s = bufs_[(size_t)slot];
		if (!s.seq) {
			int rc = grow(slot, &s, (size_t)piece_ + (size_t)piece_ / 4 + 64, (size_t)piece_ / 64 + 64, 0, 0);
			if (rc != VC_OK) return rc;
		}
		*b = s;
		return VC_OK;
	}
	int grow(int slot, VcSlotBuf *b, size_t bytes, size_t reads, size_t, size_t) override
	{
		VcSlotBuf &s = bufs_[(size_t)slot];
		uint8_t *q = (uint8_t *)realloc(s.seq, bytes);
		uint64_t *o = (uint64_t *)realloc(s.offs, reads * sizeof(uint64_t));
		uint32_t *l = (uint32_t *)realloc(s.lens, reads * sizeof(uint32_t));
		if (q) s.seq = q;
		if (o) s.offs = o;
		if (l) s.lens = l;
		if (!q || !o || !l) return VC_ENOMEM;
		s.cap_bytes = bytes;
		s.cap_reads = reads;
		*b = s;
		return VC_OK;
	}
	int submit(int, const VcSlotBuf &b, uint64_t n, uint64_t bytes) override
	{
		if (seq_out_ && nb_ + bytes <= seq_cap_) memcpy(seq_out_ + nb_, b.seq, (size_t)bytes);
		for (uint64_t i = 0; i < n; ++i)
			if (lens_out_ && nr_ + i < lens_cap_) lens_out_[nr_ + i] = b.lens[i];
		nb_ += bytes;
		nr_ += n;
		return VC_OK;
	}

private:
	std::vector<VcSlotBuf> bufs_;
	uint64_t piece_;
	uint8_t *seq_out_;
	size_t seq_cap_;
	uint32_t *lens_out_;
	size_t lens_cap_;
	uint64_t nb_ = 0, nr_ = 0;
};

double mono_now()
{
	struct timespec ts;
	clock_gettime(CLOCK_MONOTONIC, &ts);
	return ts.tv_sec + ts.tv_nsec * 1e-9;
}

}

extern "C" int vc_scan_file_parallel(const char *path, int k, int block_bases, int n_threads,
                                     uint64_t piece_bytes, vc_file_stats *st, uint8_t *seq_out, size_t seq_cap,
                                     uint32_t *lens_out, size_t lens_cap)
{
	if (!path || !st || n_threads < 1) return VC_EINVAL;
	vc_file_stats local = {0, 0, 0, 0.0};
	const double t0 = mono_now();
	struct stat sb;
	if (stat(path, &sb) != 0) return VC_EIO;
	if (!S_ISREG(sb.st_mode)) {
		VcFastqReader rd;
		if (!rd.open(path)) return VC_EIO;
		size_t nb = 0, nr = 0;
		const int rc = vc_block_loop(rd, k, block_bases, [&](const char *q, size_t l) {
			if (seq_out && nb + l <= seq_cap) memcpy(seq_out + nb, q, l);
			if (lens_out && nr < lens_cap) lens_out[nr] = (uint32_t)l;
			nb += l;
			++nr;
			return VC_OK;
		}, local);
		local.seconds = mono_now() - t0;
		*st = local;
		return rc;
	}
	const int fd = open(path, O_RDONLY);
	if (fd < 0) return VC_EIO;
	if (fstat(fd, &sb) != 0) {
		close(fd);
		return VC_EIO;
	}
	uint8_t magic[2] = {0, 0};
	if (pread_full(fd, magic, 2, 0) == 2 && magic[0] == 0x1f && magic[1] == 0x8b) {
		close(fd);
		int rc;
		VcGzParallel *g = vc_gzp_open(path, vc_gz_inflate_threads(n_threads), piece_bytes);
		if (g) {
			const uint64_t piece = vc_ingest_piece((uint64_t)16 << 20);
			const int parsers = vc_gz_parse_threads(n_threads);
			HostSink sink(parsers + 2, piece, seq_out, seq_cap, lens_out, lens_cap);
			rc = vc_ingest_gzip(g, k, block_bases, parsers, parsers + 2, piece, (uint64_t)(parsers + 4) * piece * 2,
			                    sink, local);
			vc_gzp_close(g);
		} else {
			VcFastqReader rd;
			if (!rd.open(path)) return VC_EIO;
			size_t nb = 0, nr = 0;
			rc = vc_block_loop(rd, k, block_bases, [&](const char *q, size_t l) {
				if (seq_out && nb + l <= seq_cap) memcpy(seq_out + nb, q, l);
				if (lens_out && nr < lens_cap) lens_out[nr] = (uint32_t)l;
				nb += l;
				++nr;
				return VC_OK;
			}, local);
		}
		local.seconds = mono_now() - t0;
		*st = local;
		return rc;
	}
	if (piece_bytes < 2) {
		close(fd);
		return VC_EINVAL;
	}
	const int slots = n_threads < 2 ? n_threads + 2 : 2 * n_threads;
	HostSink sink(slots, piece_bytes, seq_out, seq_cap, lens_out, lens_cap);
	const int rc = vc_ingest_plain(fd, (uint64_t)sb.st_size, k, block_bases, n_threads, slots,
	                               piece_bytes, sink, local);
	close(fd);
	local.seconds = mono_now() - t0;
	*st = local;
	return rc;
}

extern "C" int vc_scan_file_range(const char *path, int k, int block_bases, int n_threads, uint64_t piece_bytes,
                                  uint64_t begin, uint64_t end, vc_file_stats *st, vc_range_info *ri,
                                  uint8_t *seq_out, size_t seq_cap, uint32_t *lens_out, size_t lens_cap)
{
	if (!path || !st || !ri || n_threads < 1 || piece_bytes < 2 || end <= begin) return VC_EINVAL;
	vc_file_stats local = {0, 0, 0, 0.0};
	*ri = vc_range_info{UINT64_MAX, UINT64_MAX, 0, 0, 1};
	const double t0 = mono_now();
	struct stat sb;
	if (stat(path, &sb) != 0) return VC_EIO;
	const int fd = S_ISREG(sb.st_mode) ? open(path, O_RDONLY) : -1;
	if (S_ISREG(sb.st_mode) && fd < 0) return VC_EIO;
	uint8_t magic[2] = {0, 0};
	const bool reg = fd >= 0 && fstat(fd, &sb) == 0 && S_ISREG(sb.st_mode);
	if (!reg || (pread_full(fd, magic, 2, 0) == 2 && magic[0] == 0x1f && magic[1] == 0x8b)) {
		if (fd >= 0) close(fd);
		int rc = VC_OK;
		if (begin == 0) {
			rc = vc_scan_file_parallel(path, k, block_bases, n_threads, piece_bytes, &local, seq_out, seq_cap,
			                           lens_out, lens_cap);
			if (rc == VC_OK) *ri = vc_range_info{0, UINT64_MAX, 0, 1, 1};
		}
		local.seconds = mono_now() - t0;
		*st = local;
		return rc;
	}
	const int slots = n_threads < 2 ? n_threads + 2 : 2 * n_threads;
	HostSink sink(slots, piece_bytes, seq_out, seq_cap, lens_out, lens_cap);
	VcTextRange R;
	R.begin = begin;
	R.end = end;
	const int rc = vc_ingest_plain(fd, (uint64_t)sb.st_size, k, block_bases, n_threads, slots, piece_bytes, sink,
	                               local, &R);
	close(fd);
	*ri = vc_range_info{R.first, R.next, R.errs, R.stopped ? 1u : 0u, 0u};
	local.seconds = mono_now() - t0;
	*st = local;
	return rc;
}

static int scan_gz_share_g(VcGzParallel *g, int fmt, int k, int first_share, const uint8_t *window, uint64_t text_len,
                           int block_bases, int parsers, vc_file_stats &local, vc_range_info *ri,
                           vc_gz_share_crc *crc, uint8_t *seq_out, size_t seq_cap, uint32_t *lens_out,
                           size_t lens_cap)
{
	const uint64_t piece = vc_ingest_piece((uint64_t)16 << 20);
	HostSink sink(parsers + 2, piece, seq_out, seq_cap, lens_out, lens_cap);
	const size_t np = first_share ? 0 : 1;
	VcTextRange R;
	R.begin = np;
	R.end = np + text_len;
	R.format = fmt;
	const int rc = vc_ingest_gzip_share(g, first_share ? nullptr : window + 32767, np, k, block_bases, parsers,
	                                    parsers + 2, piece, (uint64_t)(parsers + 4) * piece * 2, sink, local, &R);
	VcGzShareCrc c;
	vc_gzp_share_crc(g, &c);
	vc_gzp_close(g);
	*ri = vc_range_info{R.first == UINT64_MAX ? UINT64_MAX : R.first - np,
	                    R.next == UINT64_MAX ? UINT64_MAX : R.next - np - text_len, R.errs, R.stopped ? 1u : 0u, 0u};
	*crc = vc_gz_share_crc{c.events, c.head_crc, c.head_len, c.head_expect_crc, c.head_expect_isize, c.tail_crc,
	                       c.tail_len, c.crc_error, c.complete};
	return rc;
}

extern "C" int vc_scan_gz_share(const char *path, int k, int first_share, uint64_t start_bit, const uint8_t *window,
                                uint64_t text_len, int block_bases, int n_threads, vc_file_stats *st,
                                vc_range_info *ri, vc_gz_share_crc *crc, uint8_t *seq_out, size_t seq_cap,
                                uint32_t *lens_out, size_t lens_cap)
{
	if (!path || !st || !ri || !crc || n_threads < 1 || text_len == 0 || (!first_share && !window)) return VC_EINVAL;
	vc_file_stats local = {0, 0, 0, 0.0};
	*ri = vc_range_info{UINT64_MAX, UINT64_MAX, 0, 0, 0};
	memset(crc, 0, sizeof *crc);
	const double t0 = mono_now();
	const int fmt = vc_gz_text_format(path);
	if (fmt < 0) return VC_EINVAL;
	VcGzParallel *g = vc_gzp_open_share(path, vc_gz_inflate_threads(n_threads), vc_gz_chunk(), first_share != 0,
	                                    start_bit, window, text_len);
	if (!g) return VC_EIO;
	const int rc = scan_gz_share_g(g, fmt, k, first_share, window, text_len, block_bases,
	                               vc_gz_parse_threads(n_threads), local, ri, crc, seq_out, seq_cap, lens_out,
	                               lens_cap);
	local.seconds = mono_now() - t0;
	*st = local;
	return rc;
}

extern "C" int vc_scan_gz_share_held(vc_gz_share *h, int k, int first_share, const uint8_t *window, uint64_t text_len,
                                     int block_bases, int n_threads, vc_file_stats *st, vc_range_info *ri,
                                     vc_gz_share_crc *crc, uint8_t *seq_out, size_t seq_cap, uint32_t *lens_out,
                                     size_t lens_cap)
{
	if (!h || !h->g || !st || !ri || !crc || n_threads < 1 || text_len == 0 || (!first_share && !window))
		return VC_EINVAL;
	vc_file_stats local = {0, 0, 0, 0.0};
	*ri = vc_range_info{UINT64_MAX, UINT64_MAX, 0, 0, 0};
	memset(crc, 0, sizeof *crc);
	const double t0 = mono_now();
	if (h->format < 0) return VC_EINVAL;
	VcGzParallel *g = h->g;
	h->g = nullptr;
	if (!vc_gzp_resume_share(g, first_share ? nullptr : window, text_len)) {
		vc_gzp_close(g);
		return VC_EINVAL;
	}
	const int rc = scan_gz_share_g(g, h->format, k, first_share, window, text_len, block_bases,
	                               vc_gz_held_parse_threads(n_threads), local, ri, crc, seq_out, seq_cap, lens_out,
	                               lens_cap);
	local.seconds = mono_now() - t0;
	*st = local;
	return rc;
}

extern "C" uint64_t vc_ingest_profile(double *prof)
{
	const VcIngestProfile &L = vc_ingest_last;
	if (prof) {
		prof[0] = L.total;
		prof[1] = L.main_wait;
		prof[2] = L.submit;
		prof[3] = L.reparse;
		prof[4] = L.parse;
		prof[5] = L.slot_wait;
		prof[6] = L.acquire;
	}
	return L.pieces;
}

extern "C" uint64_t vc_ingest_profile_ex(double *prof, int n)
{
	const VcIngestProfile &L = vc_ingest_last;
	const double v[VC_INGEST_PROFILE_FIELDS] = {
		L.total, L.main_wait, L.submit, L.reparse, L.parse, L.slot_wait, L.acquire, L.read_s,
		(double)L.read_bytes, L.copy_s, (double)L.copy_bytes, L.guess_s, L.worker_cpu, L.worker_wall,
		L.main_cpu, (double)L.threads, (double)L.copy_mode};
	for (int i = 0; prof && i < n && i < VC_INGEST_PROFILE_FIELDS; ++i) prof[i] = v[i];
	return L.pieces;
}
```

### kmer-cnt_amd/csrc/vafc_ingest.h

```cpp
#ifndef VAFC_INGEST_H
#define VAFC_INGEST_H

#include <stddef.h>
#include <stdint.h>
#include <stdlib.h>

#include "vafc.h"
#include "vafc_fastq.h"

template <class Sink>
inline int vc_block_loop(VcFastqReader &rd, int k, int block_bases, Sink &&sink, vc_file_stats &st)
{
	int empty = 0, rc = VC_OK;
	while (empty < 3 && rc == VC_OK) {
		int64_t sum = 0;
		int ret;
		while ((ret = rd.next()) >= 0) {
			if (ret < k) continue;
			if ((rc = sink(rd.seq(), (size_t)ret)) != VC_OK) break;
			sum += ret;
			st.bases += (uint64_t)ret;
			st.seqs += 1;
			if (sum >= block_bases) break;
		}
		if (sum == 0) ++empty;
		else ++st.blocks;
	}
	return rc;
}


struct VcSlotBuf {
	uint8_t *seq = nullptr;
	uint64_t *offs = nullptr;
	uint32_t *lens = nullptr;
	size_t cap_bytes = 0, cap_reads = 0;
};

class VcIngestSink {
public:
	virtual ~VcIngestSink() = default;
	virtual int acquire(int slot, VcSlotBuf *b) = 0;
	virtual int grow(int slot, VcSlotBuf *b, size_t bytes, size_t reads, size_t used_bytes,
	                 size_t used_reads) = 0;
	virtual int submit(int slot, const VcSlotBuf &b, uint64_t n, uint64_t bytes) = 0;
};

class VcIngestSource : public VcTextSource {
public:
	virtual bool longer_than(uint64_t off) = 0;
	virtual void release(uint64_t) {}
	virtual void abort() {}
};

struct VcTextRange {
	uint64_t begin = 0, end = UINT64_MAX;
	uint64_t first = 0, next = UINT64_MAX, errs = 0;
	bool stopped = false;
	int format = -1;
};

struct VcIngestProfile {
	double total = 0, main_wait = 0, submit = 0, reparse = 0, parse = 0, slot_wait = 0, acquire = 0;
	double read_s = 0, copy_s = 0, guess_s = 0, worker_cpu = 0, worker_wall = 0, main_cpu = 0;
	uint64_t read_bytes = 0, copy_bytes = 0;
	uint64_t pieces = 0;
	int threads = 0, copy_mode = 0;
};
extern thread_local VcIngestProfile vc_ingest_last;

int vc_ingest_text(VcIngestSource &src, int k, int block_bases, int threads, int slots, uint64_t piece_bytes,
                   VcIngestSink &sink, vc_file_stats &st, VcTextRange *range = nullptr);

int vc_ingest_plain(int fd, uint64_t size, int k, int block_bases, int threads, int slots,
                    uint64_t piece_bytes, VcIngestSink &sink, vc_file_stats &st, VcTextRange *range = nullptr);

class VcGzParallel;
inline int vc_gz_parse_threads(int threads)
{
	const char *e = getenv("VAFC_GZ_PARSERS");
	const int n = e && atoi(e) > 0 ? atoi(e) : (threads + 2) / 4;
	return n < 1 ? 1 : n;
}
inline int vc_gz_held_parse_threads(int threads)
{
	const char *e = getenv("VAFC_GZ_PARSERS");
	const int n = e && atoi(e) > 0 ? atoi(e) : threads;
	return n < 1 ? 1 : n;
}
inline int vc_gz_inflate_threads(int threads)
{
	const char *e = getenv("VAFC_GZ_INFLATERS");
	if (e && atoi(e) > 0) return atoi(e);
	return threads < 1 ? 1 : threads;
}
inline uint64_t vc_ingest_piece(uint64_t dflt)
{
	const char *e = getenv("VAFC_INGEST_PIECE");
	return e && atoll(e) >= 2 ? (uint64_t)atoll(e) : dflt;
}
inline uint64_t vc_gz_chunk()
{
	const char *e = getenv("VAFC_GZ_CHUNK");
	return e && atoll(e) > 0 ? (uint64_t)atoll(e) : 0;
}
int vc_ingest_gzip(VcGzParallel *g, int k, int block_bases, int threads, int slots, uint64_t piece_bytes,
                   uint64_t window_bytes, VcIngestSink &sink, vc_file_stats &st);
int vc_ingest_gzip_share(VcGzParallel *g, const uint8_t *prefix, size_t np, int k, int block_bases, int threads,
                         int slots, uint64_t piece_bytes, uint64_t window_bytes, VcIngestSink &sink, vc_file_stats &st,
                         VcTextRange *range);
int vc_gz_text_format(const char *path);

#endif
```

### kmer-cnt_amd/csrc/vafc_internal.h

```cpp
#ifndef VAFC_INTERNAL_H
#define VAFC_INTERNAL_H

#include <hip/hip_runtime.h>
#include <stddef.h>
#include <stdint.h>

#include "vafc_common.h"

#ifndef VC_BLOCK
#define VC_BLOCK 1024
#endif
#define VC_KV_FLANK 128
#define VC_KV_BIG 512
#define VC_QCAP 240

struct VcKernelArgs {
	const uint8_t *seq;
	uint64_t seq_words;
	uint64_t off_adj;
	const uint64_t *offs;
	const uint32_t *lens;
	uint64_t n_reads;
	const vc_slot_t *table;
	uint32_t tbits, tmask;
	const uint32_t *filter;
	uint32_t wbits;
	uint32_t fsh;
	uint32_t flank;
	uint32_t big;
	uint32_t fwords;
	uint32_t qcap;
	const uint32_t *l2f;
	uint32_t l2bits;
	int ablate;
	uint32_t variant;
	uint32_t nt4;
	int k;
	uint64_t kmask;
	uint32_t *counts;
	unsigned long long *tally;
	uint32_t *nlong;
	uint32_t *longlist;
	uint32_t long_cap;
	uint32_t *flags;
};

__host__ __device__ static inline uint32_t vc_filter_lds_words(uint32_t fwords) { return fwords + 4u; }
static inline size_t vc_lds_bytes(uint32_t fwords, uint32_t qcap)
{
	return (size_t)4 * vc_filter_lds_words(fwords) + (size_t)(VC_BLOCK / 64) * qcap * 8;
}

#ifdef __cplusplus
extern "C" {
#endif
hipError_t vc_kernel_setup(void);
hipError_t vc_launch_count(const VcKernelArgs *A, int grid, int grid_long, hipStream_t st);
hipError_t vc_launch_decode(const uint8_t *seq, uint64_t seq_bytes, const uint64_t *offs,
                            const uint32_t *lens, uint64_t n_reads, uint8_t *codes, hipStream_t st);
hipError_t vc_launch_synth(uint8_t *seq, uint64_t *offs, uint32_t *lens, uint64_t first,
                           uint64_t n_reads, uint32_t L, uint64_t seed, uint64_t thr,
                           const uint8_t *win, const uint8_t *dosage, uint32_t n_snp, hipStream_t st);
hipError_t vc_launch_shard_add(uint32_t *dst, uint32_t *src, uint64_t n, unsigned long long *dst_tally,
                               unsigned long long *src_tally, hipStream_t st);
#ifdef __cplusplus
}
#endif

#endif
```

### kmer-cnt_amd/csrc/vafc_stage.h

```cpp
#ifndef VAFC_STAGE_H
#define VAFC_STAGE_H

#include <hip/hip_runtime.h>

#include <stdint.h>
#include <stdio.h>
#include <stdlib.h>
#include <string.h>
#include <sys/mman.h>

#include <utility>

#include "vafc.h"
#include "vafc_device.h"

struct VcSlot {
	uint8_t *h_seq = nullptr;
	uint64_t *h_offs = nullptr;
	uint32_t *h_lens = nullptr;
	uint8_t *d_seq = nullptr;
	uint64_t *d_offs = nullptr;
	uint32_t *d_lens = nullptr;
	size_t cap_bytes = 0, cap_reads = 0;
	hipEvent_t done = nullptr;
	hipEvent_t copied = nullptr;
	bool pending = false;
	void *map = nullptr;
	size_t map_len = 0;
	bool d_one = false;
};

inline void vc_slot_free(VcSlot &s)
{
	if (s.map) {
		(void)hipHostUnregister(s.map);
		munmap(s.map, s.map_len);
	} else {
		if (s.h_seq) (void)hipHostFree(s.h_seq);
		if (s.h_offs) (void)hipHostFree(s.h_offs);
		if (s.h_lens) (void)hipHostFree(s.h_lens);
	}
	if (s.d_seq) (void)hipFree(s.d_seq);
	if (!s.d_one) {
		if (s.d_offs) (void)hipFree(s.d_offs);
		if (s.d_lens) (void)hipFree(s.d_lens);
	}
	const hipEvent_t done = s.done, copied = s.copied;
	s = VcSlot();
	s.done = done;
	s.copied = copied;
}

inline void vc_slot_destroy(VcSlot &s)
{
	vc_slot_free(s);
	if (s.done) (void)hipEventDestroy(s.done);
	if (s.copied) (void)hipEventDestroy(s.copied);
	s.done = s.copied = nullptr;
}

inline int vc_slot_wait(VcSlot &s)
{
	if (s.pending) HIPCK(hipEventSynchronize(s.done));
	s.pending = false;
	return VC_OK;
}

inline int vc_slot_realloc(VcSlot &s, size_t bytes, size_t reads, size_t keep_bytes, size_t keep_reads)
{
	VcSlot n;
	if (hipHostMalloc((void **)&n.h_seq, bytes, hipHostMallocDefault) != hipSuccess ||
	    hipHostMalloc((void **)&n.h_offs, reads * sizeof(uint64_t), hipHostMallocDefault) != hipSuccess ||
	    hipHostMalloc((void **)&n.h_lens, reads * sizeof(uint32_t), hipHostMallocDefault) != hipSuccess ||
	    hipMalloc((void **)&n.d_seq, bytes) != hipSuccess ||
	    hipMalloc((void **)&n.d_offs, reads * sizeof(uint64_t)) != hipSuccess ||
	    hipMalloc((void **)&n.d_lens, reads * sizeof(uint32_t)) != hipSuccess) {
		fprintf(stderr, "[E::vafc] batch buffers of %zu bytes, %zu reads: %s\n", bytes, reads,
		        hipGetErrorString(hipGetLastError()));
		vc_slot_free(n);
		return VC_EHIP;
	}
	if (keep_bytes) memcpy(n.h_seq, s.h_seq, keep_bytes);
	if (keep_reads) {
		memcpy(n.h_offs, s.h_offs, keep_reads * sizeof(uint64_t));
		memcpy(n.h_lens, s.h_lens, keep_reads * sizeof(uint32_t));
	}
	n.cap_bytes = bytes;
	n.cap_reads = reads;
	n.done = s.done;
	n.copied = s.copied;
	vc_slot_free(s);
	s = n;
	return VC_OK;
}

inline int vc_slot_reserve(VcSlot &s, size_t bytes, size_t reads)
{
	if (bytes <= s.cap_bytes && reads <= s.cap_reads) return VC_OK;
	const int rc = vc_slot_wait(s);
	if (rc != VC_OK) return rc;
	return vc_slot_realloc(s, s.cap_bytes >= bytes ? s.cap_bytes : bytes + bytes / 4 + 4096,
	                       s.cap_reads >= reads ? s.cap_reads : reads + reads / 4 + 1024, 0, 0);
}

struct VcStager {
	VcSlot slot[2];
	int cur = 0;

	int init()
	{
		for (VcSlot &s : slot) HIPCK(hipEventCreateWithFlags(&s.done, hipEventDisableTiming));
		return VC_OK;
	}
	void destroy()
	{
		for (VcSlot &s : slot) vc_slot_destroy(s);
	}
	int acquire(VcSlot **out)
	{
		*out = &slot[cur];
		return vc_slot_wait(slot[cur]);
	}
	int acquire_for(size_t bytes, size_t reads, VcSlot **out)
	{
		const int rc = acquire(out);
		return rc == VC_OK ? vc_slot_reserve(**out, bytes, reads) : rc;
	}
	template <class Launch>
	int submit(size_t bytes, uint64_t n_reads, hipStream_t st, Launch &&launch, bool per_read = true)
	{
		VcSlot &s = slot[cur];
		if (n_reads) {
			if (bytes) HIPCK(hipMemcpyAsync(s.d_seq, s.h_seq, bytes, hipMemcpyHostToDevice, st));
			if (per_read) {
				HIPCK(hipMemcpyAsync(s.d_offs, s.h_offs, n_reads * sizeof(uint64_t), hipMemcpyHostToDevice, st));
				HIPCK(hipMemcpyAsync(s.d_lens, s.h_lens, n_reads * sizeof(uint32_t), hipMemcpyHostToDevice, st));
			}
			const int rc = launch(s);
			if (rc != VC_OK) return rc;
			HIPCK(hipEventRecord(s.done, st));
			s.pending = true;
		}
		cur ^= 1;
		return VC_OK;
	}
	void settle()
	{
		for (VcSlot &s : slot) s.pending = false;
	}
};

inline size_t vc_batch_bytes(size_t dflt)
{
	const char *e = getenv("VAFC_BATCH_BYTES");
	return e && atoll(e) >= 1 ? (size_t)atoll(e) : dflt;
}

template <class Next> struct VcBatchWriter {
	size_t limit, max_reads;
	Next next;
	decltype(std::declval<Next &>()()) h = nullptr;
	VcSlot *s = nullptr;
	size_t bytes = 0;
	uint64_t n = 0;
	uint64_t batches = 0;
	int err = VC_OK;

	VcBatchWriter(size_t limit_bytes, size_t limit_reads, Next nx)
	    : limit(limit_bytes), max_reads(limit_reads ? limit_reads : 1), next(nx)
	{
	}

	int open_slot()
	{
		if (!(h = next())) return VC_EHIP;
		const int rc = h->stage.acquire_for(limit, max_reads, &s);
		if (rc != VC_OK) s = nullptr;
		bytes = 0;
		n = 0;
		return rc;
	}
	int flush()
	{
		if (!s) return VC_OK;
		const int rc = h->submit(bytes, n);
		batches += n ? 1 : 0;
		s = nullptr;
		bytes = 0;
		n = 0;
		return rc;
	}
	int add(const char *seq, size_t len)
	{
		if (!s && (err = open_slot()) != VC_OK) return err;
		if (n > 0 && (bytes + len > limit || n >= max_reads)) {
			if ((err = flush()) != VC_OK) return err;
			if ((err = open_slot()) != VC_OK) return err;
		}
		if (len > s->cap_bytes - bytes && (err = vc_slot_reserve(*s, len, 1)) != VC_OK) return err;
		if (len) memcpy(s->h_seq + bytes, seq, len);
		s->h_offs[n] = bytes;
		s->h_lens[n] = (uint32_t)len;
		bytes += len;
		++n;
		return VC_OK;
	}
};

struct VcStreamBridge {
	hipEvent_t in = nullptr, out = nullptr;

	int enter(hipStream_t own, hipStream_t st)
	{
		if (st == own) return VC_OK;
		if (!in) HIPCK(hipEventCreateWithFlags(&in, hipEventDisableTiming));
		if (!out) HIPCK(hipEventCreateWithFlags(&out, hipEventDisableTiming));
		HIPCK(hipEventRecord(in, own));
		HIPCK(hipStreamWaitEvent(st, in, 0));
		return VC_OK;
	}
	int leave(hipStream_t own, hipStream_t st)
	{
		if (st == own) return VC_OK;
		HIPCK(hipEventRecord(out, st));
		HIPCK(hipStreamWaitEvent(own, out, 0));
		return VC_OK;
	}
	void destroy()
	{
		if (in) (void)hipEventDestroy(in);
		if (out) (void)hipEventDestroy(out);
		in = out = nullptr;
	}
};

struct VcDevice {
	int dev = 0;
	int n_cu = 256;
	hipStream_t st = nullptr;
	VcStager stage;
	VcStreamBridge bridge;
	VcTimer timer;

	int open(int device)
	{
		int ndev = 0;
		if (hipGetDeviceCount(&ndev) != hipSuccess || ndev <= 0) return VC_ENODEV;
		if (device < 0 || device >= ndev) return VC_EINVAL;
		HIPCK(hipSetDevice(device));
		dev = device;
		hipDeviceProp_t prop;
		if (hipGetDeviceProperties(&prop, device) == hipSuccess && prop.multiProcessorCount > 0)
			n_cu = prop.multiProcessorCount;
		HIPCK(hipStreamCreateWithFlags(&st, hipStreamNonBlocking));
		HIPCK(timer.init());
		return stage.init();
	}
	void close()
	{
		(void)hipSetDevice(dev);
		if (st) (void)hipStreamSynchronize(st);
		stage.destroy();
		timer.destroy();
		bridge.destroy();
	}
	~VcDevice()
	{
		if (st) (void)hipStreamDestroy(st);
	}
	hipStream_t stream_of(void *stream) const { return stream == VC_STREAM_CTX ? st : (hipStream_t)stream; }
	template <class Launch> int on_stream(void *stream, Launch &&launch)
	{
		const hipStream_t s = stream_of(stream);
		int rc = bridge.enter(st, s);
		if (rc == VC_OK) rc = launch(s);
		if (rc == VC_OK) rc = bridge.leave(st, s);
		return rc;
	}
};

#endif
```

### kmer-cnt_amd/vafc.py

```python
from __future__ import annotations

import ctypes as C
import os
import sys
import time

import numpy as np

_HERE = os.path.dirname(os.path.abspath(__file__))
LIB_PATH = os.environ.get("VAFC_LIB", os.path.join(_HERE, "lib", "libvafc.so"))

STREAM_CTX = (1 << 64) - 1

VC_OK, VC_EINVAL, VC_ENOMEM, VC_EHIP, VC_ENODEV, VC_EIO, VC_ETOOMANY, VC_EFULL = 0, -1, -2, -3, -4, -5, -6, -7

EXPORTS = (
    "vc_patterns_load", "vc_patterns_free", "vc_patterns_count", "vc_patterns_keys",
    "vc_write_vaf", "vc_pattern_fields", "vc_free", "vc_create", "vc_destroy",
    "vc_count_block", "vc_count_device", "vc_finish", "vc_reset", "vc_device_counts",
    "vc_bind_outputs", "vc_device_tally", "vc_stream", "vc_set_timing", "vc_kernel_ms",
    "vc_table_info", "vc_create_multi", "vc_shard_count", "vc_shard_info", "vc_count_file",
    "vc_count_file_range", "vc_scan_file_range", "vc_ingest_profile", "vc_ingest_profile_ex", "vc_scan_file", "vc_scan_file_parallel",
    "vc_scan_records", "vc_reserve_file_ingest",
    "vc_gz_inflate_parallel", "vc_gz_inflate_zlib", "vc_gz_crc32", "vc_gz_crc32_combine",
    "vc_gz_share_scan", "vc_count_gz_share", "vc_scan_gz_share",
    "vc_gz_share_open", "vc_count_gz_share_held", "vc_scan_gz_share_held", "vc_gz_share_close",
    "vc_fasta_load", "vc_fasta_count", "vc_fasta_name", "vc_fasta_seq", "vc_fasta_data", "vc_fasta_free",
    "vc_count_candidates", "vc_set_nt4_decode",
    "vc_kc_create", "vc_kc_set_partition", "vc_kc_slots", "vc_kc_histogram", "vc_kc_histogram2",
    "vc_kc_track_first", "vc_yak_bloom_select",
    "vc_vafset_create", "vc_vafset_free", "vc_vafset_add", "vc_vafset_add_many", "vc_vafset_add_arrays",
    "vc_vafset_count",
    "vc_vafset_name", "vc_vafset_snps", "vc_corr_matrix", "vc_corr_matrix_raw", "vc_corr_write", "vc_corr_tree",
    "vc_ed_create", "vc_ed_create_raw", "vc_ed_destroy", "vc_ed_count_block", "vc_ed_count_device",
    "vc_ed_finish", "vc_ed_reset", "vc_ed_set_counts", "vc_ed_set_max_ranges", "vc_ed_shape", "vc_ed_kernel_ms",
    "vc_ed_count_file",
    "vc_bam_probe", "vc_bam_kind_name", "vc_bam_read_file", "vc_bam_read_header", "vc_bam_file_refs",
    "vc_bam_file_ref_name", "vc_bam_file_records", "vc_bam_file_free", "vc_bam_index_usable", "vc_bam_build_regions",
    "vc_bam_create", "vc_bam_destroy", "vc_bam_set_regions", "vc_bam_count_block", "vc_bam_count_device",
    "vc_bam_finish", "vc_bam_reset", "vc_bam_set_counts", "vc_bam_set_long_threshold", "vc_bam_kernel_ms",
    "vc_bam_count_file",
    "vc_vcf_probe", "vc_vcf_kind_name", "vc_vcf_header_parse", "vc_vcf_header_samples", "vc_vcf_header_type",
    "vc_vcf_header_free", "vc_vcf_eval_line", "vc_vcf_create", "vc_vcf_create_raw", "vc_vcf_destroy",
    "vc_vcf_scan_block", "vc_vcf_scan_device", "vc_vcf_hits", "vc_vcf_set_max_hits", "vc_vcf_set_block_bytes",
    "vc_vcf_kernel_ms", "vc_vcf_count_file",
    "vc_synth_reads",
    "vc_debug_decode", "vc_strerror", "vc_version", "vc_build_id",
)


class VafcError(RuntimeError):
    def __init__(self, what, code=None):
        if code is not None:
            what = "%s: %s (%d)" % (what, lib().vc_strerror(code).decode(), code)
        super().__init__(what)
        self.code = code


class FileStats(C.Structure):
    _fields_ = [("bases", C.c_uint64), ("seqs", C.c_uint64), ("blocks", C.c_uint64),
                ("seconds", C.c_double)]


class RangeInfo(C.Structure):
    _fields_ = [("first", C.c_uint64), ("next", C.c_uint64), ("errs", C.c_uint64),
                ("stopped", C.c_uint32), ("whole", C.c_uint32)]


class GzShareInfo(C.Structure):
    _fields_ = [("start_bit", C.c_uint64), ("end_bit", C.c_uint64), ("text_len", C.c_uint64),
                ("ok", C.c_uint32), ("ended", C.c_uint32)]


class GzShareCrc(C.Structure):
    _fields_ = [("events", C.c_uint32), ("head_crc", C.c_uint32), ("head_len", C.c_uint64),
                ("head_expect_crc", C.c_uint32), ("head_expect_isize", C.c_uint32), ("tail_crc", C.c_uint32),
                ("tail_len", C.c_uint64), ("crc_error", C.c_uint32), ("complete", C.c_uint32)]

    def as_dict(self):
        return {f: int(getattr(self, f)) for f, _ in self._fields_}


class VcfVerdict(C.Structure):
    _fields_ = [("verdict", C.c_int32), ("head_ok", C.c_int32), ("pos", C.c_int64), ("chrom_len", C.c_uint32),
                ("n_allele", C.c_int32), ("ref_len", C.c_uint32), ("alt_len", C.c_uint32), ("ref", C.c_uint8),
                ("alt", C.c_uint8), ("reserved", C.c_uint8 * 2), ("ref_count", C.c_uint32), ("alt_count", C.c_uint32)]


NO_OFFSET = (1 << 64) - 1
GZ_WSIZE = 32768


_lib = None
P = C.c_void_p


def lib():
    global _lib
    if _lib is not None:
        return _lib
    if not os.path.exists(LIB_PATH):
        raise VafcError("libvafc.so not built (%s); run __graft_entry__.build()" % LIB_PATH)
    if os.environ.get("VAFC_NO_TORCH", "0") != "1":
        try:
            import torch
        except ImportError:
            pass
    L = C.CDLL(LIB_PATH)
    sig = {
        "vc_patterns_load": (C.c_int, [C.c_char_p, C.POINTER(P)]),
        "vc_patterns_free": (None, [P]),
        "vc_patterns_count": (C.c_int, [P]),
        "vc_patterns_keys": (C.c_int, [P, C.c_int, C.POINTER(P), C.POINTER(P),
                                       C.POINTER(C.c_size_t), C.POINTER(C.c_int)]),
        "vc_write_vaf": (C.c_int, [P, P, C.c_char_p]),
        "vc_pattern_fields": (C.c_int, [P, C.c_int, C.POINTER(C.c_char_p), C.POINTER(C.c_int),
                                        C.POINTER(C.c_char_p), C.POINTER(C.c_char),
                                        C.POINTER(C.c_char), C.POINTER(C.c_char_p),
                                        C.POINTER(C.c_char_p)]),
        "vc_free": (None, [P]),
        "vc_create": (C.c_int, [C.POINTER(P), C.c_int, P, P, C.c_size_t, C.c_uint32, C.c_int]),
        "vc_destroy": (None, [P]),
        "vc_create_multi": (C.c_int, [C.POINTER(P), C.c_int, P, P, C.c_size_t, C.c_uint32, P, C.c_int]),
        "vc_shard_count": (C.c_int, [P]),
        "vc_shard_info": (C.c_int, [P, C.c_int, C.POINTER(C.c_int), C.POINTER(C.c_uint64)]),
        "vc_count_block": (C.c_int, [P, P, C.c_size_t, P, P, C.c_uint64]),
        "vc_count_device": (C.c_int, [P, P, C.c_size_t, P, P, C.c_uint64, P]),
        "vc_finish": (C.c_int, [P, P, C.POINTER(C.c_uint64)]),
        "vc_reset": (C.c_int, [P]),
        "vc_device_counts": (P, [P]),
        "vc_bind_outputs": (C.c_int, [P, P, P]),
        "vc_device_tally": (P, [P]),
        "vc_stream": (P, [P]),
        "vc_set_timing": (C.c_int, [P, C.c_int]),
        "vc_kernel_ms": (C.c_int, [P, C.POINTER(C.c_float)]),
        "vc_table_info": (C.c_int, [P, C.POINTER(C.c_uint64), C.POINTER(C.c_uint64),
                                    C.POINTER(C.c_uint64)]),
        "vc_count_file": (C.c_int, [P, C.c_char_p, C.c_int, C.c_int, C.POINTER(FileStats)]),
        "vc_count_file_range": (C.c_int, [P, C.c_char_p, C.c_uint64, C.c_uint64, C.c_int, C.c_int,
                                          C.POINTER(FileStats), C.POINTER(RangeInfo)]),
        "vc_scan_file_range": (C.c_int, [C.c_char_p, C.c_int, C.c_int, C.c_int, C.c_uint64, C.c_uint64,
                                         C.c_uint64, C.POINTER(FileStats), C.POINTER(RangeInfo), P, C.c_size_t,
                                         P, C.c_size_t]),
        "vc_ingest_profile": (C.c_uint64, [P]),
        "vc_ingest_profile_ex": (C.c_uint64, [P, C.c_int]),
        "vc_scan_file": (C.c_int, [C.c_char_p, C.c_int, C.c_int, C.POINTER(FileStats), P, C.c_size_t,
                                   P, C.c_size_t]),
        "vc_scan_file_parallel": (C.c_int, [C.c_char_p, C.c_int, C.c_int, C.c_int, C.c_uint64,
                                            C.POINTER(FileStats), P, C.c_size_t, P, C.c_size_t]),
        "vc_scan_records": (C.c_int64, [C.c_char_p, P, C.c_int64]),
        "vc_gz_inflate_parallel": (C.c_int64, [C.c_char_p, C.c_int, C.c_uint64, P, C.c_uint64, P]),
        "vc_gz_inflate_zlib": (C.c_int64, [C.c_char_p, P, C.c_uint64]),
        "vc_gz_crc32": (C.c_uint32, [C.c_uint32, P, C.c_uint64]),
        "vc_gz_crc32_combine": (C.c_uint32, [C.c_uint32, C.c_uint32, C.c_uint64]),
        "vc_gz_share_scan": (C.c_int, [C.c_char_p, C.c_uint64, C.c_uint64, C.c_int, C.c_uint64,
                                       C.POINTER(GzShareInfo), P]),
        "vc_count_gz_share": (C.c_int, [P, C.c_char_p, C.c_int, C.c_uint64, P, C.c_uint64, C.c_int, C.c_int,
                                        C.POINTER(FileStats), C.POINTER(RangeInfo), C.POINTER(GzShareCrc)]),
        "vc_scan_gz_share": (C.c_int, [C.c_char_p, C.c_int, C.c_int, C.c_uint64, P, C.c_uint64, C.c_int, C.c_int,
                                       C.POINTER(FileStats), C.POINTER(RangeInfo), C.POINTER(GzShareCrc),
                                       P, C.c_size_t, P, C.c_size_t]),
        "vc_gz_share_open": (C.c_int, [P, C.c_char_p, C.c_uint64, C.c_uint64, C.c_int, C.c_uint64, C.c_uint64,
                                       C.POINTER(GzShareInfo), P, C.POINTER(P)]),
        "vc_count_gz_share_held": (C.c_int, [P, P, C.c_int, P, C.c_uint64, C.c_int, C.c_int, C.POINTER(FileStats),
                                             C.POINTER(RangeInfo), C.POINTER(GzShareCrc)]),
        "vc_scan_gz_share_held": (C.c_int, [P, C.c_int, C.c_int, P, C.c_uint64, C.c_int, C.c_int,
                                            C.POINTER(FileStats), C.POINTER(RangeInfo), C.POINTER(GzShareCrc),
                                            P, C.c_size_t, P, C.c_size_t]),
        "vc_gz_share_close": (None, [P]),
        "vc_reserve_file_ingest": (C.c_int, [P, C.c_int]),
        "vc_fasta_load": (C.c_int, [C.c_char_p, C.POINTER(P)]),
        "vc_fasta_count": (C.c_int, [P]),
        "vc_fasta_name": (C.c_char_p, [P, C.c_int]),
        "vc_fasta_seq": (P, [P, C.c_int, C.POINTER(C.c_uint32)]),
        "vc_fasta_data": (C.c_int, [P, C.POINTER(P), C.POINTER(C.c_size_t), C.POINTER(P), C.POINTER(P)]),
        "vc_fasta_free": (None, [P]),
        "vc_set_nt4_decode": (C.c_int, [P, C.c_int]),
        "vc_count_candidates": (C.c_int, [C.c_int, P, C.c_size_t, P, P, C.c_uint64, P, C.c_size_t, P,
                                          C.c_int]),
        "vc_kc_create": (C.c_int, [C.POINTER(P), C.c_int, C.c_uint64, C.c_int]),
        "vc_kc_set_partition": (C.c_int, [P, C.c_uint32, C.c_uint32]),
        "vc_kc_slots": (C.c_uint64, [P]),
        "vc_kc_histogram": (C.c_int, [P, P, C.POINTER(C.c_uint64), C.POINTER(C.c_uint64)]),
        "vc_kc_histogram2": (C.c_int, [P, P, C.c_uint32, C.c_uint64, C.POINTER(C.c_uint64),
                                       C.POINTER(C.c_uint64)]),
        "vc_kc_track_first": (C.c_int, [P, C.c_int]),
        "vc_yak_bloom_select": (C.c_int, [P, C.c_int, C.c_int, C.c_int]),
        "vc_vafset_create": (C.c_int, [C.POINTER(P)]),
        "vc_vafset_free": (None, [P]),
        "vc_vafset_add": (C.c_int, [P, C.c_char_p]),
        "vc_vafset_add_many": (C.c_int, [P, P, C.c_int, C.c_int, C.POINTER(C.c_int), P]),
        "vc_vafset_add_arrays": (C.c_int, [P, C.c_char_p, P, P, C.c_int]),
        "vc_vafset_count": (C.c_int, [P]),
        "vc_vafset_name": (C.c_char_p, [P, C.c_int]),
        "vc_vafset_snps": (C.c_int, [P, C.c_int]),
        "vc_corr_matrix": (C.c_int, [P, C.c_int, C.c_int, P, C.c_int, C.POINTER(C.c_float)]),
        "vc_corr_matrix_raw": (C.c_int, [P, P, P, C.c_int, C.c_size_t, C.c_int, C.c_int, P, C.c_int,
                                         C.POINTER(C.c_float)]),
        "vc_corr_write": (C.c_int, [P, P, C.c_char_p]),
        "vc_corr_tree": (C.c_int, [P, P, C.c_char_p]),
        "vc_ed_create": (C.c_int, [C.POINTER(P), P, C.c_int, C.c_int]),
        "vc_ed_create_raw": (C.c_int, [C.POINTER(P), P, P, P, C.c_size_t, C.c_int, C.c_int]),
        "vc_ed_destroy": (None, [P]),
        "vc_ed_count_block": (C.c_int, [P, P, C.c_size_t, P, P, C.c_uint64]),
        "vc_ed_count_device": (C.c_int, [P, P, C.c_size_t, P, P, C.c_uint64, P]),
        "vc_ed_finish": (C.c_int, [P, P]),
        "vc_ed_reset": (C.c_int, [P]),
        "vc_ed_set_counts": (C.c_int, [P, P]),
        "vc_ed_set_max_ranges": (C.c_int, [P, C.c_uint32]),
        "vc_ed_shape": (C.c_int, [P, C.c_int, C.POINTER(C.c_uint32), C.POINTER(C.c_int), C.POINTER(C.c_int)]),
        "vc_ed_kernel_ms": (C.c_int, [P, C.POINTER(C.c_float)]),
        "vc_ed_count_file": (C.c_int, [P, C.c_char_p, C.c_int, C.POINTER(FileStats)]),
        "vc_bam_probe": (C.c_int, [C.c_char_p, C.POINTER(C.c_int)]),
        "vc_bam_kind_name": (C.c_char_p, [C.c_int]),
        "vc_bam_read_file": (C.c_int, [C.c_char_p, C.c_int, C.POINTER(P)]),
        "vc_bam_read_header": (C.c_int, [C.c_char_p, C.POINTER(P)]),
        "vc_bam_file_refs": (C.c_int, [P]),
        "vc_bam_file_ref_name": (C.c_char_p, [P, C.c_int]),
        "vc_bam_file_records": (C.c_uint64, [P, C.POINTER(P), C.POINTER(P), C.POINTER(C.c_uint64)]),
        "vc_bam_file_free": (None, [P]),
        "vc_bam_index_usable": (C.c_int, [C.c_char_p, C.c_char_p, C.c_size_t]),
        "vc_bam_build_regions": (C.c_int, [P, P, P]),
        "vc_bam_create": (C.c_int, [C.POINTER(P), P, C.POINTER(C.c_char_p), C.c_int, C.c_int]),
        "vc_bam_destroy": (None, [P]),
        "vc_bam_set_regions": (C.c_int, [P, P, P, P, C.c_size_t]),
        "vc_bam_count_block": (C.c_int, [P, P, C.c_uint64, P, C.c_size_t]),
        "vc_bam_count_device": (C.c_int, [P, P, C.c_uint64, P, C.c_size_t, P]),
        "vc_bam_finish": (C.c_int, [P, P]),
        "vc_bam_reset": (C.c_int, [P]),
        "vc_bam_set_counts": (C.c_int, [P, P]),
        "vc_bam_set_long_threshold": (C.c_int, [P, C.c_uint32]),
        "vc_bam_kernel_ms": (C.c_int, [P, C.POINTER(C.c_float)]),
        "vc_bam_count_file": (C.c_int, [P, C.c_char_p, C.c_int, C.POINTER(FileStats)]),
        "vc_vcf_probe": (C.c_int, [C.c_char_p, C.POINTER(C.c_int)]),
        "vc_vcf_kind_name": (C.c_char_p, [C.c_int]),
        "vc_vcf_header_parse": (C.c_int, [P, C.c_size_t, C.c_int, C.POINTER(P), C.POINTER(C.c_size_t)]),
        "vc_vcf_header_samples": (C.c_int, [P]),
        "vc_vcf_header_type": (C.c_int, [P, C.c_char_p]),
        "vc_vcf_header_free": (None, [P]),
        "vc_vcf_eval_line": (C.c_int, [P, P, C.c_size_t, C.c_int, C.c_int, C.POINTER(VcfVerdict)]),
        "vc_vcf_create": (C.c_int, [C.POINTER(P), P, C.c_int]),
        "vc_vcf_create_raw": (C.c_int, [C.POINTER(P), C.POINTER(C.c_char_p), P, P, P, C.c_size_t, C.c_size_t, C.c_int]),
        "vc_vcf_destroy": (None, [P]),
        "vc_vcf_scan_block": (C.c_int, [P, P, C.c_size_t, C.c_uint64, C.c_int, C.POINTER(C.c_size_t)]),
        "vc_vcf_scan_device": (C.c_int, [P, P, C.c_size_t, C.c_uint64, C.c_int, P]),
        "vc_vcf_hits": (C.c_int, [P, C.POINTER(P), C.POINTER(C.c_size_t), C.POINTER(C.c_size_t)]),
        "vc_vcf_set_max_hits": (C.c_int, [P, C.c_size_t]),
        "vc_vcf_set_block_bytes": (C.c_int, [P, C.c_size_t]),
        "vc_vcf_kernel_ms": (C.c_int, [P, C.POINTER(C.c_float)]),
        "vc_vcf_count_file": (C.c_int, [P, C.c_char_p, C.c_int, C.c_int, C.c_int, P, C.POINTER(FileStats)]),
        "vc_synth_reads": (C.c_int, [P, P, P, C.c_uint64, C.c_uint64, C.c_uint32, C.c_uint64,
                                     C.c_double, P, P, C.c_uint32, P]),
        "vc_debug_decode": (C.c_int, [P, C.c_size_t, P, P, C.c_uint64, P, P]),
        "vc_strerror": (C.c_char_p, [C.c_int]),
        "vc_version": (C.c_int, []),
        "vc_build_id": (C.c_char_p, []),
    }
    older = "VAFC_LIB" in os.environ
    for name, (res, args) in sig.items():
        if older and not hasattr(L, name):
            continue
        f = getattr(L, name)
        f.restype = res
        f.argtypes = args
    _lib = L
    return L


def tree_build_id(root: str = None) -> str:
    import hashlib
    csrc = os.path.join(_HERE, "csrc")
    root = root or os.path.dirname(_HERE)
    h = hashlib.sha256()
    for fn in sorted(os.listdir(csrc)):
        p = os.path.join(csrc, fn)
        if os.path.isfile(p):
            with open(p, "rb") as f:
                h.update(f.read())
    with open(os.path.join(root, "include", "vafc.h"), "rb") as f:
        h.update(f.read())
    return h.hexdigest()[:16]


def binary_build_id(path: str):
    import re
    try:
        with open(path, "rb") as f:
            m = re.search(rb"VAFC_BUILD_ID=([0-9a-f]{16})", f.read())
    except OSError:
        return None
    return m.group(1).decode() if m else None


def check_build(paths=None) -> None:
    want = tree_build_id()
    lib_dir = os.path.join(_HERE, "lib")
    paths = paths or [os.path.join(lib_dir, f) for f in BINARIES]
    bad = [(os.path.basename(p), binary_build_id(p)) for p in paths if binary_build_id(p) != want]
    if bad:
        raise VafcError("stale or missing build: the tree's sources hash to %s, but %s; "
                        "rebuild with make -C kmer-cnt_amd/csrc" % (
                            want, ", ".join("%s has %s" % (n, i) for n, i in bad)))


BINARIES = ("libvafc.so", "vaf-counter", "snp-pattern-gen", "kc-c4", "yak-count", "correlation-matrix",
            "ed-vaf-counter", "bam-vaf-counter", "vcf-vaf-counter")


def _ck(rc, what):
    if rc != VC_OK:
        raise VafcError(what, rc)


def _ptr(a: np.ndarray):
    return a.ctypes.data_as(P)



class PatternDB:

    def __init__(self, handle):
        self._h = handle

    @property
    def n(self) -> int:
        return lib().vc_patterns_count(self._h)

    def __len__(self):
        return self.n

    def record(self, i: int):
        chr_, rsid, rk, ak = C.c_char_p(), C.c_char_p(), C.c_char_p(), C.c_char_p()
        start, ref, alt = C.c_int(), C.c_char(), C.c_char()
        _ck(lib().vc_pattern_fields(self._h, i, C.byref(chr_), C.byref(start), C.byref(rsid),
                                    C.byref(ref), C.byref(alt), C.byref(rk), C.byref(ak)),
            "vc_pattern_fields")
        return (chr_.value.decode("latin-1"), start.value, rsid.value.decode("latin-1"),
                ref.value, alt.value, rk.value, ak.value)

    def keys(self, k: int):
        kp, vp, n, coll = P(), P(), C.c_size_t(), C.c_int()
        _ck(lib().vc_patterns_keys(self._h, k, C.byref(kp), C.byref(vp), C.byref(n), C.byref(coll)),
            "vc_patterns_keys")
        try:
            m = n.value
            keys = np.ctypeslib.as_array(C.cast(kp, C.POINTER(C.c_uint64)), (m,)).copy() if m else \
                np.zeros(0, np.uint64)
            vals = np.ctypeslib.as_array(C.cast(vp, C.POINTER(C.c_uint32)), (m,)).copy() if m else \
                np.zeros(0, np.uint32)
        finally:
            lib().vc_free(kp)
            lib().vc_free(vp)
        return keys, vals, coll.value

    def write_vaf(self, counts: np.ndarray, path: str) -> None:
        counts = np.ascontiguousarray(counts, dtype=np.uint32)
        assert counts.size >= 2 * self.n
        _ck(lib().vc_write_vaf(self._h, _ptr(counts), path.encode()), "vc_write_vaf")

    def close(self):
        if self._h:
            lib().vc_patterns_free(self._h)
            self._h = None

    def __del__(self):
        try:
            self.close()
        except Exception:
            pass


def load_patterns(fn: str) -> PatternDB:
    h = P()
    _ck(lib().vc_patterns_load(fn.encode(), C.byref(h)), "load_patterns(%s)" % fn)
    return PatternDB(h)



class KmerMap:

    def __init__(self, k: int, keys: np.ndarray, vals: np.ndarray, n_patterns: int, device: int = 0,
                 devices=None):
        keys = np.ascontiguousarray(keys, dtype=np.uint64)
        vals = np.ascontiguousarray(vals, dtype=np.uint32)
        self.k, self.n_patterns, self.device = k, int(n_patterns), device
        h = P()
        if devices:
            devs = np.ascontiguousarray(devices, dtype=np.int32)
            self.device = int(devs[0])
            _ck(lib().vc_create_multi(C.byref(h), k, _ptr(keys), _ptr(vals), keys.size, self.n_patterns,
                                      _ptr(devs), devs.size), "vc_create_multi")
        else:
            _ck(lib().vc_create(C.byref(h), k, _ptr(keys), _ptr(vals), keys.size, self.n_patterns, device),
                "vc_create")
        self._h = h
        self.n_collisions = 0

    def shards(self):
        out = []
        for i in range(lib().vc_shard_count(self._h)):
            d, b = C.c_int(), C.c_uint64()
            _ck(lib().vc_shard_info(self._h, i, C.byref(d), C.byref(b)), "vc_shard_info")
            out.append((d.value, b.value))
        return out

    def count_block(self, seq: np.ndarray, offs: np.ndarray, lens: np.ndarray) -> None:
        seq = np.ascontiguousarray(seq, dtype=np.uint8)
        offs = np.ascontiguousarray(offs, dtype=np.uint64)
        lens = np.ascontiguousarray(lens, dtype=np.uint32)
        assert offs.size == lens.size
        _ck(lib().vc_count_block(self._h, _ptr(seq), seq.size, _ptr(offs), _ptr(lens), offs.size),
            "vc_count_block")

    def count_device(self, seq_ptr: int, seq_bytes: int, offs_ptr: int, lens_ptr: int,
                     n_reads: int, stream: int = 0) -> None:
        _ck(lib().vc_count_device(self._h, P(seq_ptr), seq_bytes, P(offs_ptr), P(lens_ptr),
                                  n_reads, P(stream) if stream else None), "vc_count_device")

    def reserve_file_ingest(self, n_thread: int = 4) -> None:
        _ck(lib().vc_reserve_file_ingest(self._h, n_thread), "vc_reserve_file_ingest")

    def count_file(self, fn: str, block_size: int = 10_000_000, n_thread: int = 4) -> FileStats:
        st = FileStats()
        rc = lib().vc_count_file(self._h, fn.encode(), block_size, n_thread, C.byref(st))
        if rc == VC_EIO:
            raise FileNotFoundError(fn)
        _ck(rc, "vc_count_file(%s)" % fn)
        return st

    def count_gz_share(self, fn: str, first_share: bool, start_bit: int, window, text_len: int,
                       block_size: int = 10_000_000, n_thread: int = 4):
        st, ri, cr = FileStats(), RangeInfo(), GzShareCrc()
        w = None if window is None else np.ascontiguousarray(window, dtype=np.uint8)
        rc = lib().vc_count_gz_share(self._h, fn.encode(), 1 if first_share else 0, start_bit,
                                     None if w is None else _ptr(w), text_len, block_size, n_thread,
                                     C.byref(st), C.byref(ri), C.byref(cr))
        if rc == VC_EIO:
            raise FileNotFoundError(fn)
        _ck(rc, "vc_count_gz_share(%s)" % fn)
        return st, ri, cr.as_dict()

    def count_gz_share_held(self, share, first_share: bool, window, text_len: int, block_size: int = 10_000_000,
                            n_thread: int = 4):
        st, ri, cr = FileStats(), RangeInfo(), GzShareCrc()
        w = None if window is None else np.ascontiguousarray(window, dtype=np.uint8)
        rc = lib().vc_count_gz_share_held(self._h, share.handle(), 1 if first_share else 0,
                                          None if w is None else _ptr(w), text_len, block_size, n_thread,
                                          C.byref(st), C.byref(ri), C.byref(cr))
        _ck(rc, "vc_count_gz_share_held")
        return st, ri, cr.as_dict()

    def count_file_range(self, fn: str, begin: int, end: int, block_size: int = 10_000_000,
                         n_thread: int = 4):
        st, ri = FileStats(), RangeInfo()
        rc = lib().vc_count_file_range(self._h, fn.encode(), begin, min(end, NO_OFFSET), block_size, n_thread,
                                       C.byref(st), C.byref(ri))
        if rc == VC_EIO:
            raise FileNotFoundError(fn)
        _ck(rc, "vc_count_file_range(%s)" % fn)
        return st, ri

    def finish(self):
        counts = np.zeros(2 * self.n_patterns + 2, dtype=np.uint32)
        km = C.c_uint64()
        _ck(lib().vc_finish(self._h, _ptr(counts), C.byref(km)), "vc_finish")
        return counts[:2 * self.n_patterns], km.value

    def reset(self) -> None:
        _ck(lib().vc_reset(self._h), "vc_reset")

    def bind_outputs(self, counts_ptr: int = 0, tally_ptr: int = 0) -> None:
        _ck(lib().vc_bind_outputs(self._h, P(counts_ptr) if counts_ptr else None,
                                  P(tally_ptr) if tally_ptr else None), "vc_bind_outputs")

    @property
    def stream(self) -> int:
        return lib().vc_stream(self._h) or 0

    def set_timing(self, on: bool = True) -> None:
        _ck(lib().vc_set_timing(self._h, 1 if on else 0), "vc_set_timing")

    def kernel_ms(self) -> float:
        ms = C.c_float()
        _ck(lib().vc_kernel_ms(self._h, C.byref(ms)), "vc_kernel_ms")
        return ms.value

    def table_info(self):
        a, b, c = C.c_uint64(), C.c_uint64(), C.c_uint64()
        _ck(lib().vc_table_info(self._h, C.byref(a), C.byref(b), C.byref(c)), "vc_table_info")
        return {"n_keys": a.value, "slots": b.value, "filter_bytes": c.value}

    def close(self):
        if getattr(self, "_h", None):
            lib().vc_destroy(self._h)
            self._h = None

    def __del__(self):
        try:
            self.close()
        except Exception:
            pass


def create_combined_kmer_map(db: PatternDB, k: int, device: int = 0, devices=None) -> KmerMap:
    keys, vals, coll = db.keys(k)
    if coll > 0:
        sys.stderr.write("[W::create_combined_kmer_map] Warning: %d k-mer collisions detected. "
                         "Some patterns may have overlapping k-mers.\n" % coll)
    m = KmerMap(k, keys, vals, db.n, device, devices)
    m.n_collisions = coll
    return m


def count_fastq_kmers(fn: str, k: int, n_thread: int, block_size: int, kmer_map: KmerMap,
                      db: PatternDB = None):
    assert k == kmer_map.k
    try:
        return kmer_map.count_file(fn, block_size, n_thread)
    except FileNotFoundError:
        return None


def scan_file(fn: str, k: int, block_size: int = 10_000_000, with_reads: bool = False):
    st = FileStats()
    if not with_reads:
        rc = lib().vc_scan_file(fn.encode(), k, block_size, C.byref(st), None, 0, None, 0)
        reads = None
    else:
        size = _text_size(fn) + 16
        seq = np.zeros(max(size * 4, 64), np.uint8)
        lens = np.zeros(max(size, 16), np.uint32)
        rc = lib().vc_scan_file(fn.encode(), k, block_size, C.byref(st), _ptr(seq), seq.size,
                                _ptr(lens), lens.size)
        reads = []
        pos = 0
        for i in range(int(st.seqs)):
            n = int(lens[i])
            reads.append(seq[pos:pos + n].tobytes())
            pos += n
    if rc == VC_EIO:
        raise FileNotFoundError(fn)
    _ck(rc, "vc_scan_file")
    return st, reads


def _text_size(fn: str) -> int:
    with open(fn, "rb") as f:
        gz = f.read(2) == b"\x1f\x8b"
    if not gz:
        return os.path.getsize(fn)
    n = lib().vc_gz_inflate_zlib(fn.encode(), None, 0)
    return max(int(n), 0)


def gz_inflate_parallel(fn: str, threads: int = 4, chunk_bytes: int = 4 << 20):
    st = np.zeros(6, np.uint64)
    n = lib().vc_gz_inflate_parallel(fn.encode(), threads, chunk_bytes, None, 0, _ptr(st))
    if n < 0:
        return None
    cap = int(n) + 1
    out = np.zeros(cap, np.uint8)
    n = lib().vc_gz_inflate_parallel(fn.encode(), threads, chunk_bytes, _ptr(out), cap, _ptr(st))
    keys = ("chunks", "accepted", "skipped", "fallback", "members", "crc_error")
    return out[:min(int(n), cap)].tobytes(), dict(zip(keys, (int(x) for x in st)))


def gz_inflate_zlib(fn: str) -> bytes:
    cap = _text_size(fn) + 1
    out = np.zeros(cap, np.uint8)
    n = lib().vc_gz_inflate_zlib(fn.encode(), _ptr(out), cap)
    if n < 0:
        raise FileNotFoundError(fn)
    return out[:int(n)].tobytes()


def scan_file_parallel(fn: str, k: int, block_size: int = 10_000_000, threads: int = 4,
                       piece_bytes: int = 8 << 20, with_reads: bool = False):
    st = FileStats()
    if not with_reads:
        rc = lib().vc_scan_file_parallel(fn.encode(), k, block_size, threads, piece_bytes, C.byref(st),
                                         None, 0, None, 0)
        reads = None
    else:
        size = _text_size(fn) + 16
        seq = np.zeros(max(size, 64), np.uint8)
        lens = np.zeros(max(size, 16), np.uint32)
        rc = lib().vc_scan_file_parallel(fn.encode(), k, block_size, threads, piece_bytes, C.byref(st),
                                         _ptr(seq), seq.size, _ptr(lens), lens.size)
        reads = []
        pos = 0
        for i in range(int(st.seqs)):
            n = int(lens[i])
            reads.append(seq[pos:pos + n].tobytes())
            pos += n
    if rc == VC_EIO:
        raise FileNotFoundError(fn)
    _ck(rc, "vc_scan_file_parallel")
    return st, reads


def scan_file_range(fn: str, k: int, begin: int, end: int, block_size: int = 10_000_000, threads: int = 4,
                    piece_bytes: int = 8 << 20, with_reads: bool = False):
    st, ri = FileStats(), RangeInfo()
    end = min(end, NO_OFFSET)
    if not with_reads:
        rc = lib().vc_scan_file_range(fn.encode(), k, block_size, threads, piece_bytes, begin, end, C.byref(st),
                                      C.byref(ri), None, 0, None, 0)
        reads = None
    else:
        size = _text_size(fn) + 16
        seq = np.zeros(max(size, 64), np.uint8)
        lens = np.zeros(max(size, 16), np.uint32)
        rc = lib().vc_scan_file_range(fn.encode(), k, block_size, threads, piece_bytes, begin, end, C.byref(st),
                                      C.byref(ri), _ptr(seq), seq.size, _ptr(lens), lens.size)
        reads = []
        pos = 0
        for i in range(int(st.seqs)):
            n = int(lens[i])
            reads.append(seq[pos:pos + n].tobytes())
            pos += n
    if rc == VC_EIO:
        raise FileNotFoundError(fn)
    _ck(rc, "vc_scan_file_range")
    return st, ri, reads


def gz_share_scan(fn: str, begin: int, end: int, threads: int = 4, chunk_bytes: int = 0):
    info = GzShareInfo()
    wsym = np.zeros(GZ_WSIZE, np.uint16)
    rc = lib().vc_gz_share_scan(fn.encode(), begin, min(end, NO_OFFSET), threads, chunk_bytes, C.byref(info),
                                _ptr(wsym))
    if rc == VC_EIO:
        raise FileNotFoundError(fn)
    _ck(rc, "vc_gz_share_scan(%s)" % fn)
    return {f: int(getattr(info, f)) for f, _ in info._fields_}, wsym


class GzShare:

    def __init__(self, h):
        self._h = h

    def handle(self):
        if not self._h:
            raise VafcError("gz share already closed")
        return self._h

    def close(self):
        if self._h:
            lib().vc_gz_share_close(self._h)
            self._h = None

    def __del__(self):
        try:
            self.close()
        except Exception:
            pass


def gz_share_open(fn: str, begin: int, end: int, threads: int = 4, chunk_bytes: int = 0, hold_bytes: int = 0,
                  kmap=None):
    info = GzShareInfo()
    wsym = np.zeros(GZ_WSIZE, np.uint16)
    h = P()
    rc = lib().vc_gz_share_open(None if kmap is None else kmap._h, fn.encode(), begin, min(end, NO_OFFSET), threads, chunk_bytes, hold_bytes,
                                C.byref(info), _ptr(wsym), C.byref(h))
    if rc == VC_EIO:
        raise FileNotFoundError(fn)
    _ck(rc, "vc_gz_share_open(%s)" % fn)
    return {f: int(getattr(info, f)) for f, _ in info._fields_}, wsym, (GzShare(h.value) if h.value else None)


def gz_window_after(wsym: np.ndarray, before: np.ndarray) -> np.ndarray:
    w = np.asarray(wsym, dtype=np.uint16)
    b = np.asarray(before, dtype=np.uint8)
    return np.where(w < 256, w, b[w & (GZ_WSIZE - 1)]).astype(np.uint8)


def gz_crc32_combine(crc1: int, crc2: int, len2: int) -> int:
    return int(lib().vc_gz_crc32_combine(crc1, crc2, len2))


def scan_gz_share(fn: str, k: int, first_share: bool, start_bit: int, window, text_len: int,
                  block_size: int = 10_000_000, threads: int = 4, with_reads: bool = False, cap: int = 0):
    st, ri, cr = FileStats(), RangeInfo(), GzShareCrc()
    w = None if window is None else np.ascontiguousarray(window, dtype=np.uint8)
    seq = lens = None
    if with_reads:
        n = max(cap or 2 * text_len + 4096, 64)
        seq = np.zeros(n, np.uint8)
        lens = np.zeros(max(n // 2, 16), np.uint32)
    rc = lib().vc_scan_gz_share(fn.encode(), k, 1 if first_share else 0, start_bit, None if w is None else _ptr(w),
                                text_len, block_size, threads, C.byref(st), C.byref(ri), C.byref(cr),
                                None if seq is None else _ptr(seq), 0 if seq is None else seq.size,
                                None if lens is None else _ptr(lens), 0 if lens is None else lens.size)
    if rc == VC_EIO:
        raise FileNotFoundError(fn)
    _ck(rc, "vc_scan_gz_share(%s)" % fn)
    reads = None
    if with_reads:
        reads, pos = [], 0
        for i in range(int(st.seqs)):
            m = int(lens[i])
            reads.append(seq[pos:pos + m].tobytes())
            pos += m
    return st, ri, cr.as_dict(), reads


def scan_gz_share_held(share, k: int, first_share: bool, window, text_len: int, block_size: int = 10_000_000,
                       threads: int = 4, with_reads: bool = False, cap: int = 0):
    st, ri, cr = FileStats(), RangeInfo(), GzShareCrc()
    w = None if window is None else np.ascontiguousarray(window, dtype=np.uint8)
    seq = lens = None
    if with_reads:
        n = max(cap or 2 * text_len + 4096, 64)
        seq = np.zeros(n, np.uint8)
        lens = np.zeros(max(n // 2, 16), np.uint32)
    rc = lib().vc_scan_gz_share_held(share.handle(), k, 1 if first_share else 0, None if w is None else _ptr(w),
                                     text_len, block_size, threads, C.byref(st), C.byref(ri), C.byref(cr),
                                     None if seq is None else _ptr(seq), 0 if seq is None else seq.size,
                                     None if lens is None else _ptr(lens), 0 if lens is None else lens.size)
    _ck(rc, "vc_scan_gz_share_held")
    reads = None
    if with_reads:
        reads, pos = [], 0
        for i in range(int(st.seqs)):
            m = int(lens[i])
            reads.append(seq[pos:pos + m].tobytes())
            pos += m
    return st, ri, cr.as_dict(), reads


INGEST_PROFILE_KEYS = ("reader_s", "main_wait_s", "submit_s", "reparse_s", "parse_thread_s", "slot_wait_thread_s",
                       "acquire_thread_s", "read_thread_s", "read_bytes", "copy_thread_s", "copy_bytes",
                       "guess_thread_s", "worker_cpu_s", "worker_wall_s", "main_cpu_s", "threads", "copy_mode")


def ingest_profile() -> dict:
    out = np.zeros(len(INGEST_PROFILE_KEYS), np.float64)
    n = lib().vc_ingest_profile_ex(_ptr(out), len(out))
    d = {k: round(float(v), 4) for k, v in zip(INGEST_PROFILE_KEYS, out)}
    for k in ("read_bytes", "copy_bytes", "threads", "copy_mode"):
        d[k] = int(d[k])
    d["pieces"] = int(n)
    return d


def scan_records(fn: str, cap: int = 1 << 20) -> np.ndarray:
    rets = np.zeros(cap, np.int32)
    n = lib().vc_scan_records(fn.encode(), _ptr(rets), cap)
    if n == VC_EIO:
        raise FileNotFoundError(fn)
    return rets[:min(n, cap)]


def synth_reads(seq_ptr, offs_ptr, lens_ptr, first, n_reads, read_len, seed, f_snp,
                windows_ptr, dosage_ptr, n_snp, stream=0) -> None:
    _ck(lib().vc_synth_reads(P(seq_ptr), P(offs_ptr), P(lens_ptr), first, n_reads, read_len, seed,
                             f_snp, P(windows_ptr) if n_snp else None,
                             P(dosage_ptr) if n_snp else None, n_snp,
                             P(stream) if stream else None), "vc_synth_reads")


def debug_decode(seq_ptr, seq_bytes, offs_ptr, lens_ptr, n_reads, codes_ptr, stream=0) -> None:
    _ck(lib().vc_debug_decode(P(seq_ptr), seq_bytes, P(offs_ptr), P(lens_ptr), n_reads,
                              P(codes_ptr), P(stream) if stream else None), "vc_debug_decode")



USAGE = (
    "Usage: vaf-counter [options] -p <patterns.txt> -o <output.vaf> <reads.fq> [reads2.fq ...]\n"
    "Options:\n"
    "  -k INT    k-mer length [%d]\n"
    "  -p FILE   input pattern file\n"
    "  -o FILE   output VAF file\n"
    "  -t INT    number of threads [%d]\n"
    "  -b INT    block size [%d]\n"
    "  -v        verbose mode (report performance statistics)\n")


def parse_args(argv):
    opt = {"k": 21, "t": 4, "b": 10_000_000, "p": None, "o": None, "v": False}
    files, i = [], 0
    while i < len(argv):
        a = argv[i]
        if a == "--":
            files.extend(argv[i + 1:])
            break
        if len(a) >= 2 and a[0] == "-":
            j = 1
            while j < len(a):
                c = a[j]
                if c in "kpotb":
                    val = a[j + 1:] if j + 1 < len(a) else (argv[i + 1] if i + 1 < len(argv) else None)
                    if j + 1 >= len(a):
                        i += 1
                    if val is not None:
                        if c in "ktb":
                            try:
                                opt[c] = int(val)
                            except ValueError:
                                opt[c] = 0
                        else:
                            opt[c] = val
                    break
                if c == "v":
                    opt["v"] = True
                j += 1
        else:
            files.append(a)
        i += 1
    return opt, files


def main(argv=None) -> int:
    argv = sys.argv[1:] if argv is None else argv
    o, files = parse_args(argv)
    k = o["k"]
    if not o["p"] or not o["o"] or not files:
        sys.stderr.write(USAGE % (k, o["t"], o["b"]))
        return 1
    err = sys.stderr.write
    t_start = time.time()
    err("[M::main] Loading patterns...\n")
    t = time.time()
    try:
        db = load_patterns(o["p"])
    except VafcError:
        err("Error: failed to load pattern file\n")
        return 1
    err("[M::main] Loaded %d patterns in %.3f sec\n" % (db.n, time.time() - t))
    err("[M::main] Creating k-mer map...\n")
    try:
        devs = [int(x) for x in os.environ.get("VAFC_DEVICES", "").split(",") if x.strip()]
        kmap = create_combined_kmer_map(db, k, int(os.environ.get("VAFC_DEVICE", "0")), devs or None)
    except VafcError:
        err("Error: failed to create k-mer map\n")
        return 1
    err("[M::main] Counting k-mers in FASTQ files with %d threads...\n" % o["t"])
    t = time.time()
    bases = seqs = 0
    for fn in files:
        err("[M::main] Processing %s...\n" % fn)
        st = count_fastq_kmers(fn, k, o["t"], o["b"], kmap, db)
        if st is not None:
            bases += st.bases
            seqs += st.seqs
    counts, kmers = kmap.finish()
    t_count = time.time() - t
    tot = int(counts.astype(np.uint64).sum())
    avg = tot / (db.n if db.n > 0 else 1)
    err("[M::main] Writing VAF file...\n")
    try:
        db.write_vaf(counts, o["o"])
    except VafcError:
        err("Error: failed to open output file\n")
        return 1
    err("[M::main] Done. Average depth: %.2f\n" % avg)
    if o["v"]:
        err("  Bases processed:       %d (%.2f Mbases)\n" % (bases, bases / 1e6))
        err("  K-mers extracted:      %d (%.2f million)\n" % (kmers, kmers / 1e6))
        if t_count > 0:
            err("  Speed:                 %.2f Mbases/sec\n" % (bases / t_count / 1e6))
        err("  Total runtime:         %.3f sec\n" % (time.time() - t_start))
    kmap.close()
    db.close()
    return 0


if __name__ == "__main__":
    sys.exit(main())



def load_fasta(fn: str):
    h = P()
    rc = lib().vc_fasta_load(fn.encode(), C.byref(h))
    if rc == VC_EIO:
        raise FileNotFoundError(fn)
    _ck(rc, "vc_fasta_load")
    try:
        out = []
        for i in range(lib().vc_fasta_count(h)):
            n = C.c_uint32()
            p = lib().vc_fasta_seq(h, i, C.byref(n))
            out.append((lib().vc_fasta_name(h, i), C.string_at(p, n.value) if n.value else b""))
        return out
    finally:
        lib().vc_fasta_free(h)


def count_candidate_kmers(k: int, seqs, keys, device: int = 0) -> np.ndarray:
    seqs = [bytes(s) for s in seqs]
    blob = np.frombuffer(b"".join(seqs), np.uint8) if any(seqs) else np.zeros(1, np.uint8)
    lens = np.array([len(s) for s in seqs], np.uint32)
    offs = np.concatenate([[0], np.cumsum(lens, dtype=np.uint64)[:-1]]).astype(np.uint64) if len(seqs) else \
        np.zeros(1, np.uint64)
    keys = np.ascontiguousarray(keys, np.uint64)
    counts = np.zeros(max(keys.size, 1), np.uint32)
    blob = np.ascontiguousarray(blob)
    _ck(lib().vc_count_candidates(k, _ptr(blob), int(sum(len(s) for s in seqs)), _ptr(offs), _ptr(lens),
                                  len(seqs), _ptr(keys), keys.size, _ptr(counts), device),
        "vc_count_candidates")
    return counts[:keys.size]



class KmerHistogram(KmerMap):

    def __init__(self, k: int, slots: int = 0, device: int = 0):
        self.k, self.n_patterns, self.device = k, 0, device
        h = P()
        _ck(lib().vc_kc_create(C.byref(h), k, slots, device), "vc_kc_create")
        self._h = h
        self.n_collisions = 0

    @property
    def slots(self) -> int:
        return lib().vc_kc_slots(self._h)

    def set_partition(self, n_parts: int, part: int) -> None:
        _ck(lib().vc_kc_set_partition(self._h, n_parts, part), "vc_kc_set_partition")

    def histogram(self, n_bins: int = 256, min_count: int = 1):
        hist = np.zeros(n_bins, np.uint64)
        d, km = C.c_uint64(), C.c_uint64()
        _ck(lib().vc_kc_histogram2(self._h, _ptr(hist), n_bins, min_count, C.byref(d), C.byref(km)),
            "vc_kc_histogram2")
        return hist, d.value, km.value

    def track_first(self, on: bool = True) -> None:
        _ck(lib().vc_kc_track_first(self._h, 1 if on else 0), "vc_kc_track_first")

    def yak_bloom_select(self, pre: int, bf_shift: int, n_hash: int) -> None:
        _ck(lib().vc_yak_bloom_select(self._h, pre, bf_shift, n_hash), "vc_yak_bloom_select")


def kc_count_file(fn: str, k: int = 31, block_size: int = 10_000_000, n_thread: int = 4,
                  slots: int = 0, device: int = 0) -> np.ndarray:
    h = KmerHistogram(k, slots, device)
    try:
        n_parts = 1
        while True:
            total = np.zeros(256, np.uint64)
            kmers, full = 0, False
            for part in range(n_parts):
                h.set_partition(n_parts, part)
                h.count_file(fn, block_size, n_thread)
                h.finish()
                try:
                    hist, _, kmers = h.histogram()
                except VafcError as e:
                    if e.code != VC_EFULL:
                        raise
                    full = True
                    break
                total += hist
            if not full:
                return total
            cap = h.slots * 7 // 10
            n_parts = max(n_parts * 2, -(-kmers // cap) if cap else 2)
            if n_parts > 1024:
                raise VafcError("k-mer table too small", VC_EFULL)
    finally:
        h.close()


def kc_main(argv=None) -> int:
    import getopt
    argv = sys.argv[1:] if argv is None else argv
    k, p, b, t = 31, 10, 10_000_000, 4
    try:
        opts, args = getopt.gnu_getopt(argv, "k:p:b:t:")
    except getopt.GetoptError:
        opts, args = [], []
    for o, v in opts:
        if o == "-k":
            k = int(v)
        elif o == "-p":
            p = int(v)
        elif o == "-b":
            b = int(v)
        elif o == "-t":
            t = int(v)
    if not args:
        sys.stderr.write("Usage: kc-c4 [options] <in.fa>\nOptions:\n"
                         "  -k INT     k-mer size [%d]\n  -p INT     prefix length [%d]\n"
                         "  -b INT     block size [%d]\n  -t INT     number of worker threads [%d]\n"
                         % (k, p, b, t))
        return 1
    if p < 10:
        sys.stderr.write("ERROR: -p should be at least 10\n")
        return 1
    hist = kc_count_file(args[0], k, b, t, int(os.environ.get("VAFC_KC_SLOTS", "0")),
                         int(os.environ.get("VAFC_DEVICE", "0")))
    sys.stdout.write("".join("%d\t%d\n" % (i, hist[i]) for i in range(1, 256)))
    return 0


def yak_count_file(fn1: str, fn2: str = None, k: int = 31, pre: int = 10, bf_shift: int = 0, n_hash: int = 4,
                   chunk_size: int = 10_000_000, n_thread: int = 4, slots: int = 0, device: int = 0):
    fn2 = fn1 if fn2 is None else fn2
    two_pass = bf_shift > 0
    replay = two_pass and fn1 != fn2
    block = min(chunk_size, 0x7FFFFFFF)
    h = KmerHistogram(k, slots, device)
    try:
        n_parts = 1
        while True:
            total, tot, kmers, full = np.zeros(1024, np.uint64), 0, 0, False
            for part in range(n_parts):
                h.set_partition(n_parts, part)
                if replay:
                    h.track_first(True)
                h.count_file(fn1, block, n_thread)
                h.finish()
                try:
                    if replay:
                        h.yak_bloom_select(pre, bf_shift, n_hash)
                        h.count_file(fn2, block, n_thread)
                        h.finish()
                    hist, d, kmers = h.histogram(1024, 2 if two_pass else 1)
                except VafcError as e:
                    if e.code != VC_EFULL:
                        raise
                    full = True
                    break
                total += hist
                tot += d
            if not full:
                return total, tot
            cap = h.slots * 7 // 10
            n_parts = max(n_parts * 2, -(-kmers // cap) if cap else 2)
            if n_parts > 1024:
                raise VafcError("k-mer table too small", VC_EFULL)
    finally:
        h.close()


def yak_main(argv=None) -> int:
    import getopt
    argv = sys.argv[1:] if argv is None else argv
    k, pre, chunk, t, b, H = 31, 10, 10_000_000, 4, 0, 4
    try:
        opts, args = getopt.gnu_getopt(argv, "k:p:K:t:b:H:")
    except getopt.GetoptError:
        opts, args = [], []
    for o, v in opts:
# ... 533 lines not shown
```

Baseline: 40070.

## Pack bases into nibbles on host and unpack on GPU to halve H2D traffic

The ingest workers now encode each base (ACGTNU, upper or lower case) as a 4-bit code using an AVX2 packer while staging into pinned memory. The device sink copies the half-size packed buffer and runs a new unpack kernel before the counting kernel. Pieces containing other characters fall back to the plain copy path by reparsing, and packing is turned off after 8 fallbacks. This cuts host write bandwidth and PCIe bytes at the cost of extra CPU packing work, an extra kernel launch and extra device memory per slot.

```diff
diff --git a/include/vafc.h b/include/vafc.h
--- a/include/vafc.h
+++ b/include/vafc.h
@@ -105,6 +105,11 @@
 
 #define VC_INGEST_PROFILE_FIELDS 17
 uint64_t vc_ingest_profile_ex(double *prof, int n);
+
+void vc_ingest_pack_stats(uint64_t *packed_pieces, uint64_t *fallback_pieces);
+int64_t vc_pack_nibbles(const uint8_t *src, size_t n, uint8_t *dst, uint32_t *state, int last, int impl);
+void vc_unpack_nibbles_host(const uint8_t *packed, size_t n, uint8_t *out);
+int vc_unpack_device(const void *d_packed, uint64_t n, void *d_out, void *stream);
 
 int vc_reserve_file_ingest(vc_ctx *ctx, int n_threads);
 
diff --git a/kmer-cnt_amd/csrc/vafc_host.cpp b/kmer-cnt_amd/csrc/vafc_host.cpp
--- a/kmer-cnt_amd/csrc/vafc_host.cpp
+++ b/kmer-cnt_amd/csrc/vafc_host.cpp
@@ -706,6 +706,7 @@
 		int rc = vc_slot_wait(s);
 		if (rc != VC_OK) return rc;
 		if (!s.h_seq || s.cap_bytes < ingest_slot_bytes(piece_)) rc = ingest_slot_alloc(s, piece_);
+		if (rc == VC_OK) rc = vc_slot_ensure_pack(s);
 		if (rc == VC_OK) fill(s, b);
 		return rc;
 	}
@@ -714,22 +715,26 @@
 		vc_ctx *sh;
 		VcSlot &s = at(slot, &sh);
 		HIPCK(hipSetDevice(sh->dev));
-		const int rc = vc_slot_realloc(s, bytes, reads, used_bytes, used_reads);
+		int rc = vc_slot_realloc(s, bytes, reads, used_bytes, used_reads);
+		if (rc == VC_OK) rc = vc_slot_ensure_pack(s);
 		if (rc == VC_OK) fill(s, b);
 		return rc;
 	}
-	int submit(int slot, const VcSlotBuf &, uint64_t n, uint64_t bytes) override
+	bool packs() const override { return true; }
+	int submit(int slot, const VcSlotBuf &, uint64_t n, uint64_t bytes, bool packed) override
 	{
 		vc_ctx *sh;
 		VcSlot &s = at(slot, &sh);
 		HIPCK(hipSetDevice(sh->dev));
 		if (!sh->cst) HIPCK(hipStreamCreateWithFlags(&sh->cst, hipStreamNonBlocking));
 		if (!s.copied) HIPCK(hipEventCreateWithFlags(&s.copied, hipEventDisableTiming));
-		HIPCK(hipMemcpyAsync(s.d_seq, s.h_seq, bytes, hipMemcpyHostToDevice, sh->cst));
+		if (packed) HIPCK(hipMemcpyAsync(s.d_pack, s.h_seq, (bytes + 1) / 2, hipMemcpyHostToDevice, sh->cst));
+		else HIPCK(hipMemcpyAsync(s.d_seq, s.h_seq, bytes, hipMemcpyHostToDevice, sh->cst));
 		HIPCK(hipMemcpyAsync(s.d_offs, s.h_offs, n * sizeof(uint64_t), hipMemcpyHostToDevice, sh->cst));
 		HIPCK(hipMemcpyAsync(s.d_lens, s.h_lens, n * sizeof(uint32_t), hipMemcpyHostToDevice, sh->cst));
 		HIPCK(hipEventRecord(s.copied, sh->cst));
 		HIPCK(hipStreamWaitEvent(sh->st, s.copied, 0));
+		if (packed) HIPCK(vc_launch_unpack(s.d_pack, bytes, s.d_seq, sh->n_cu, sh->st));
 		int rc = launch(sh, s.d_seq, bytes, s.d_offs, s.d_lens, n, sh->st, any_long(s.h_lens, n));
 		if (rc != VC_OK) return rc;
 		HIPCK(hipEventRecord(s.done, sh->st));
@@ -789,6 +794,7 @@
 	const size_t huge = (size_t)2 << 20;
 	const size_t ob = (bytes + 63) / 64 * 64, lb = ob + reads * sizeof(uint64_t);
 	const size_t need = lb + reads * sizeof(uint32_t);
+	const size_t pb = (need + 63) / 64 * 64, dneed = pb + bytes / 2 + 64;
 	const size_t len = (need + huge - 1) / huge * huge;
 	void *m = mmap(nullptr, len + huge, PROT_READ | PROT_WRITE, MAP_PRIVATE | MAP_ANONYMOUS, -1, 0);
 	if (m == MAP_FAILED) return VC_ENOMEM;
@@ -804,7 +810,7 @@
 		return VC_EHIP;
 	}
 	uint8_t *d = nullptr;
-	if (hipMalloc(&d, need) != hipSuccess) {
+	if (hipMalloc(&d, dneed) != hipSuccess) {
 		(void)hipGetLastError();
 		(void)hipHostUnregister(a);
 		munmap(a, len);
@@ -819,6 +825,7 @@
 	s.d_offs = (uint64_t *)(d + ob);
 	s.d_lens = (uint32_t *)(d + lb);
 	s.d_one = true;
+	s.d_pack = d + pb;
 	s.cap_bytes = bytes;
 	s.cap_reads = reads;
 	return VC_OK;
diff --git a/kmer-cnt_amd/csrc/vafc_ingest.cpp b/kmer-cnt_amd/csrc/vafc_ingest.cpp
--- a/kmer-cnt_amd/csrc/vafc_ingest.cpp
+++ b/kmer-cnt_amd/csrc/vafc_ingest.cpp
@@ -33,6 +33,7 @@
 	VcSlotBuf buf;
 	int rc = VC_OK;
 	bool ready = false;
+	bool packed = false;
 };
 
 double ing_clock(clockid_t id)
@@ -60,36 +61,158 @@
 	return (ssize_t)got;
 }
 
-int slot_copy_mode()
+int slot_copy_mode(bool sink_packs)
 {
 	const char *e = getenv("VAFC_SLOT_COPY");
-	return e && e[0] >= '0' && e[0] <= '2' ? e[0] - '0' : 2;
+	const int m = e && e[0] >= '0' && e[0] <= '3' ? e[0] - '0' : (sink_packs ? 3 : 2);
+	return m == 3 && !sink_packs ? 2 : m;
+}
+
+
+struct NibbleTables {
+	uint8_t code[256];
+	uint8_t letter[16];
+	NibbleTables()
+	{
+		memset(code, 0xFF, sizeof code);
+		memset(letter, 0, sizeof letter);
+		const char *up = "ACGTNU";
+		for (int c = 0; c < 6; ++c) {
+			code[(uint8_t)up[c]] = (uint8_t)c;
+			code[(uint8_t)(up[c] | 0x20)] = (uint8_t)(c | 8);
+			letter[c] = (uint8_t)up[c];
+			letter[c | 8] = (uint8_t)(up[c] | 0x20);
+		}
+	}
+};
+const NibbleTables nib_tab;
+
+bool pack_pairs_scalar(const uint8_t *s, size_t n, uint8_t *d)
+{
+	unsigned bad = 0;
+	for (size_t i = 0; i < n; i += 2) {
+		const unsigned a = nib_tab.code[s[i]], b = nib_tab.code[s[i + 1]];
+		bad |= a | b;
+		d[i >> 1] = (uint8_t)(a | (b << 4));
+	}
+	return !(bad & 0x80);
+}
+
+__attribute__((target("avx2"))) bool pack_pairs_avx2(const uint8_t *s, size_t n, uint8_t *d)
+{
+	const __m256i lut_code = _mm256_setr_epi8(0, 0, 0, 1, 3, 5, 0, 2, 0, 0, 0, 0, 0, 0, 4, 0,
+	                                          0, 0, 0, 1, 3, 5, 0, 2, 0, 0, 0, 0, 0, 0, 4, 0);
+	const char X = (char)0xFF;
+	const __m256i lut_let = _mm256_setr_epi8(X, 'A', X, 'C', 'T', 'U', X, 'G', X, X, X, X, X, X, 'N', X,
+	                                         X, 'A', X, 'C', 'T', 'U', X, 'G', X, X, X, X, X, X, 'N', X);
+	const __m256i m0f = _mm256_set1_epi8(0x0F), mdf = _mm256_set1_epi8((char)0xDF), m20 = _mm256_set1_epi8(0x20);
+	const __m256i mul = _mm256_set1_epi16(0x1001);
+	__m256i ok = _mm256_set1_epi8((char)0xFF);
+	size_t i = 0;
+	for (; i + 64 <= n; i += 64) {
+		const __m256i a = _mm256_loadu_si256((const __m256i *)(s + i));
+		const __m256i b = _mm256_loadu_si256((const __m256i *)(s + i + 32));
+		const __m256i la = _mm256_and_si256(a, m0f), lb = _mm256_and_si256(b, m0f);
+		ok = _mm256_and_si256(ok, _mm256_cmpeq_epi8(_mm256_and_si256(a, mdf), _mm256_shuffle_epi8(lut_let, la)));
+		ok = _mm256_and_si256(ok, _mm256_cmpeq_epi8(_mm256_and_si256(b, mdf), _mm256_shuffle_epi8(lut_let, lb)));
+		const __m256i ca = _mm256_or_si256(_mm256_shuffle_epi8(lut_code, la),
+		                                   _mm256_srli_epi16(_mm256_and_si256(a, m20), 2));
+		const __m256i cb = _mm256_or_si256(_mm256_shuffle_epi8(lut_code, lb),
+		                                   _mm256_srli_epi16(_mm256_and_si256(b, m20), 2));
+		const __m256i p = _mm256_packus_epi16(_mm256_maddubs_epi16(ca, mul), _mm256_maddubs_epi16(cb, mul));
+		_mm256_storeu_si256((__m256i *)(d + (i >> 1)), _mm256_permute4x64_epi64(p, 0xD8));
+	}
+	const bool tail_ok = pack_pairs_scalar(s + i, n - i, d + (i >> 1));
+	return tail_ok && _mm256_movemask_epi8(ok) == -1;
+}
+
+enum { PACK_AUTO = 0, PACK_SCALAR = 1, PACK_AVX2 = 2 };
+
+bool pack_pairs(const uint8_t *s, size_t n, uint8_t *d, int impl = PACK_AUTO)
+{
+	static const bool avx2 = __builtin_cpu_supports("avx2");
+	return (impl == PACK_AUTO ? avx2 : impl == PACK_AVX2) ? pack_pairs_avx2(s, n, d) : pack_pairs_scalar(s, n, d);
+}
+
+struct NibblePacker {
+	bool has = false;
+	uint8_t carry = 0;
+	int64_t feed(const uint8_t *s, size_t n, uint8_t *d, int impl = PACK_AUTO)
+	{
+		size_t w = 0;
+		if (!n) return 0;
+		if (has) {
+			const uint8_t c = nib_tab.code[*s];
+			if (c == 0xFF) return -1;
+			d[w++] = (uint8_t)(carry | (c << 4));
+			has = false;
+			++s;
+			--n;
+		}
+		const size_t even = n & ~(size_t)1;
+		if (!pack_pairs(s, even, d + w, impl)) return -1;
+		w += even >> 1;
+		if (n & 1) {
+			const uint8_t c = nib_tab.code[s[n - 1]];
+			if (c == 0xFF) return -1;
+			carry = c;
+			has = true;
+		}
+		return (int64_t)w;
+	}
+	size_t end(uint8_t *d)
+	{
+		if (!has) return 0;
+		*d = carry;
+		has = false;
+		return 1;
+	}
+};
+
+void unpack_nibbles(const uint8_t *p, size_t n, uint8_t *out)
+{
+	for (size_t i = 0; i < n; ++i) out[i] = nib_tab.letter[(p[i >> 1] >> ((i & 1) * 4)) & 15];
 }
 
 class SlotCopier {
 public:
 	explicit SlotCopier(int mode) : mode_(mode) {}
-	void bind(uint8_t *dst) { dst_ = dst; }
+	void set_mode(int mode) { mode_ = mode; }
+	void bind(uint8_t *dst)
+	{
+		dst_ = dst;
+		pk_ = NibblePacker();
+		wr_ = 0;
+		foreign_ = false;
+	}
+	void rebind(uint8_t *dst) { dst_ = dst; }
+	bool foreign() const { return foreign_; }
 	void add(const char *src, size_t len, uint64_t at, bool in_window)
 	{
 		if (mode_ == 0) {
 			memcpy(dst_ + at, src, len);
 			return;
 		}
-		if (!in_window || len > kStage / 2) {
+		const size_t room = mode_ == 3 ? 2 * kStage : kStage;
+		if (!in_window || len > room / 2) {
 			flush();
 			const double t0 = ing_clock(CLOCK_MONOTONIC);
-			memcpy(dst_ + at, src, len);
+			if (mode_ == 3) {
+				for (size_t i = 0; i < len && !foreign_; i += room)
+					pack((const uint8_t *)src + i, len - i < room ? len - i : room);
+			} else {
+				memcpy(dst_ + at, src, len);
+			}
 			secs += ing_clock(CLOCK_MONOTONIC) - t0;
 			bytes += len;
 			return;
 		}
-		if (!ents_.empty() && (pend_ + len > kStage || at != d1_)) flush();
+		if (!ents_.empty() && (pend_ + len > room || at != d1_)) flush();
 		if (ents_.empty()) d0_ = d1_ = at;
 		ents_.push_back({(const uint8_t *)src, (uint32_t)len});
 		d1_ += len;
 		pend_ += len;
-		if (pend_ >= kStage / 2) flush();
+		if (pend_ >= room / 2) flush();
 	}
 	void flush()
 	{
@@ -101,6 +224,17 @@
 				memcpy(d, e.src, e.len);
 				d += e.len;
 			}
+		} else if (mode_ == 3) {
+			uint8_t *s = stage_;
+			for (const Ent &e : ents_) {
+				const int64_t w = foreign_ ? -1 : pk_.feed(e.src, e.len, s);
+				if (w < 0) {
+					foreign_ = true;
+					break;
+				}
+				s += w;
+			}
+			if (!foreign_) put((size_t)(s - stage_));
 		} else {
 			uint8_t *s = stage_;
 			for (const Ent &e : ents_) {
@@ -117,7 +251,8 @@
 	void finish()
 	{
 		flush();
-		if (mode_ == 2) _mm_sfence();
+		if (mode_ == 3 && !foreign_) put(pk_.end(stage_));
+		if (mode_ >= 2) _mm_sfence();
 	}
 	static void refill_hook(void *self) { ((SlotCopier *)self)->flush(); }
 	double secs = 0;
@@ -134,7 +269,22 @@
 	std::vector<Ent> ents_;
 	uint64_t d0_ = 0, d1_ = 0;
 	size_t pend_ = 0;
-	alignas(64) uint8_t stage_[kStage];
+	NibblePacker pk_;
+	uint64_t wr_ = 0;
+	bool foreign_ = false;
+	alignas(64) uint8_t stage_[kStage + 64];
+
+	void pack(const uint8_t *s, size_t n)
+	{
+		const int64_t w = pk_.feed(s, n, stage_);
+		if (w < 0) foreign_ = true;
+		else put((size_t)w);
+	}
+	void put(size_t n)
+	{
+		stream(dst_ + wr_, stage_, n);
+		wr_ += n;
+	}
 
 	__attribute__((target("avx2"))) static void stream_avx2(uint8_t *d, const uint8_t *s, size_t n)
 	{
@@ -417,6 +567,8 @@
 		if (g >= 0 || at_eof || want == cap) return g;
 	}
 }
+
+constexpr int kForeign = 1;
 
 int parse_piece(VcTextSource &src, uint64_t start, int k, int slot, VcIngestSink &sink, VcFastqReader &rd,
                 Piece &P, SlotCopier &cp)
@@ -473,16 +625,38 @@
 			cp.flush();
 			int rc = sink.grow(slot, &P.buf, nb, nr, used, (size_t)P.n);
 			if (rc != VC_OK) return rc;
-			cp.bind(P.buf.seq);
+			cp.rebind(P.buf.seq);
 		}
 		cp.add(rd.seq(), len, used, rd.seq_in_window());
+		if (cp.foreign()) return kForeign;
 		P.buf.offs[P.n] = used;
 		P.buf.lens[P.n] = (uint32_t)len;
 		used += len;
 		P.bytes += len;
 		++P.n;
 	}
-	return VC_OK;
+	cp.finish();
+	return cp.foreign() ? kForeign : VC_OK;
+}
+
+struct StagePolicy {
+	explicit StagePolicy(int m) : mode(m) {}
+	const int mode;
+	std::atomic<int> fallbacks{0};
+	bool pack_next() const { return mode == 3 && fallbacks.load(std::memory_order_relaxed) < 8; }
+};
+
+int stage_piece(VcTextSource &src, uint64_t start, int k, int slot, VcIngestSink &sink, VcFastqReader &rd,
+                Piece &P, SlotCopier &cp, StagePolicy &pol)
+{
+	P.packed = pol.pack_next();
+	cp.set_mode(P.packed ? 3 : (pol.mode == 3 ? 2 : pol.mode));
+	const int rc = parse_piece(src, start, k, slot, sink, rd, P, cp);
+	if (rc != kForeign) return rc;
+	pol.fallbacks.fetch_add(1, std::memory_order_relaxed);
+	P.packed = false;
+	cp.set_mode(2);
+	return parse_piece(src, start, k, slot, sink, rd, P, cp);
 }
 
 struct BlockState {
@@ -541,7 +715,9 @@
                    VcIngestSink &sink, vc_file_stats &st, VcTextRange *range)
 {
 	const bool prof_print = getenv("VAFC_INGEST_PROFILE") != nullptr;
-	const int copy_mode = slot_copy_mode();
+	const int copy_mode = slot_copy_mode(sink.packs());
+	StagePolicy pol(copy_mode);
+	uint64_t n_packed = 0;
 	vc_ingest_last = VcIngestProfile();
 	double t_wait = 0, t_submit = 0, t_reparse = 0;
 	std::atomic<uint64_t> t_parse_us{0}, t_slotwait_us{0}, t_acquire_us{0};
@@ -613,7 +789,7 @@
 				const double g0 = ing_now();
 				const int64_t g = P.a == 0 ? 0 : guess_record(src, P.a, fasta, tmp);
 				w_guess_ns += (uint64_t)((ing_now() - g0) * 1e9);
-				if (g >= 0) rc = parse_piece(src, (uint64_t)g, k, slot, sink, rd, P, cp);
+				if (g >= 0) rc = stage_piece(src, (uint64_t)g, k, slot, sink, rd, P, cp, pol);
 				else P.start = -1;
 			}
 			{
@@ -680,7 +856,7 @@
 		if (rc == VC_OK && !S.stopped && P.b > expect) {
 			if (P.start < 0 || (uint64_t)P.start != expect) {
 				const double r0 = ing_now();
-				rc = parse_piece(src, expect, k, slot, sink, rd, P, mcp);
+				rc = stage_piece(src, expect, k, slot, sink, rd, P, mcp, pol);
 				t_reparse += ing_now() - r0;
 			}
 			if (rc == VC_OK) {
@@ -690,7 +866,8 @@
 				if (keep) {
 					const uint64_t bytes = (uint64_t)P.buf.offs[keep - 1] + P.buf.lens[keep - 1];
 					const double s0 = ing_now();
-					rc = sink.submit(slot, P.buf, keep, bytes);
+					rc = sink.submit(slot, P.buf, keep, bytes, P.packed);
+					n_packed += P.packed ? 1 : 0;
 					t_submit += ing_now() - s0;
 				}
 			}
@@ -729,6 +906,8 @@
 		L.worker_wall = w_wall_ns.load() * 1e-9;
 		L.main_cpu = ing_clock(CLOCK_THREAD_CPUTIME_ID) - main_cpu0;
 		L.copy_mode = copy_mode;
+		L.packed_pieces = n_packed;
+		L.fallback_pieces = (uint64_t)pol.fallbacks.load();
 	}
 	if (prof_print) {
 		const VcIngestProfile &L = vc_ingest_last;
@@ -805,7 +984,12 @@
 public:
 	HostSink(int slots, uint64_t piece, uint8_t *seq_out, size_t seq_cap, uint32_t *lens_out, size_t lens_cap)
 		: bufs_((size_t)slots), piece_(piece), seq_out_(seq_out), seq_cap_(seq_cap), lens_out_(lens_out),
-		  lens_cap_(lens_cap) {}
+		  lens_cap_(lens_cap)
+	{
+		const char *e = getenv("VAFC_SCAN_PACK");
+		packs_ = e && e[0] == '1';
+	}
+	bool packs() const override { return packs_; }
 	~HostSink() override
 	{
 		for (auto &b : bufs_) {
@@ -839,9 +1023,12 @@
 		*b = s;
 		return VC_OK;
 	}
-	int submit(int, const VcSlotBuf &b, uint64_t n, uint64_t bytes) override
-	{
-		if (seq_out_ && nb_ + bytes <= seq_cap_) memcpy(seq_out_ + nb_, b.seq, (size_t)bytes);
+	int submit(int, const VcSlotBuf &b, uint64_t n, uint64_t bytes, bool packed) override
+	{
+		if (seq_out_ && nb_ + bytes <= seq_cap_) {
+			if (packed) unpack_nibbles(b.seq, (size_t)bytes, seq_out_ + nb_);
+			else memcpy(seq_out_ + nb_, b.seq, (size_t)bytes);
+		}
 		for (uint64_t i = 0; i < n; ++i)
 			if (lens_out_ && nr_ + i < lens_cap_) lens_out_[nr_ + i] = b.lens[i];
 		nb_ += bytes;
@@ -857,6 +1044,7 @@
 	uint32_t *lens_out_;
 	size_t lens_cap_;
 	uint64_t nb_ = 0, nr_ = 0;
+	bool packs_ = false;
 };
 
 double mono_now()
@@ -1078,3 +1266,29 @@
 	for (int i = 0; prof && i < n && i < VC_INGEST_PROFILE_FIELDS; ++i) prof[i] = v[i];
 	return L.pieces;
 }
+
+extern "C" void vc_ingest_pack_stats(uint64_t *packed_pieces, uint64_t *fallback_pieces)
+{
+	if (packed_pieces) *packed_pieces = vc_ingest_last.packed_pieces;
+	if (fallback_pieces) *fallback_pieces = vc_ingest_last.fallback_pieces;
+}
+
+
+extern "C" int64_t vc_pack_nibbles(const uint8_t *src, size_t n, uint8_t *dst, uint32_t *state, int last, int impl)
+{
+	if (!dst || !state || (n && !src) || impl < PACK_AUTO || impl > PACK_AVX2) return VC_EINVAL;
+	if (impl == PACK_AVX2 && !__builtin_cpu_supports("avx2")) return VC_ENODEV;
+	NibblePacker pk;
+	pk.has = (*state & 0x100u) != 0;
+	pk.carry = (uint8_t)(*state & 15u);
+	int64_t w = pk.feed(src, n, dst, impl);
+	if (w < 0) return VC_EINVAL;
+	if (last) w += (int64_t)pk.end(dst + w);
+	*state = pk.has ? 0x100u | pk.carry : 0u;
+	return w;
+}
+
+extern "C" void vc_unpack_nibbles_host(const uint8_t *packed, size_t n, uint8_t *out)
+{
+	if (packed && out) unpack_nibbles(packed, n, out);
+}
diff --git a/kmer-cnt_amd/csrc/vafc_ingest.h b/kmer-cnt_amd/csrc/vafc_ingest.h
--- a/kmer-cnt_amd/csrc/vafc_ingest.h
+++ b/kmer-cnt_amd/csrc/vafc_ingest.h
@@ -43,7 +43,8 @@
 	virtual int acquire(int slot, VcSlotBuf *b) = 0;
 	virtual int grow(int slot, VcSlotBuf *b, size_t bytes, size_t reads, size_t used_bytes,
 	                 size_t used_reads) = 0;
-	virtual int submit(int slot, const VcSlotBuf &b, uint64_t n, uint64_t bytes) = 0;
+	virtual int submit(int slot, const VcSlotBuf &b, uint64_t n, uint64_t bytes, bool packed) = 0;
+	virtual bool packs() const { return false; }
 };
 
 class VcIngestSource : public VcTextSource {
@@ -66,6 +67,7 @@
 	uint64_t read_bytes = 0, copy_bytes = 0;
 	uint64_t pieces = 0;
 	int threads = 0, copy_mode = 0;
+	uint64_t packed_pieces = 0, fallback_pieces = 0;
 };
 extern thread_local VcIngestProfile vc_ingest_last;
 
diff --git a/kmer-cnt_amd/csrc/vafc_internal.h b/kmer-cnt_amd/csrc/vafc_internal.h
--- a/kmer-cnt_amd/csrc/vafc_internal.h
+++ b/kmer-cnt_amd/csrc/vafc_internal.h
@@ -61,6 +61,7 @@
 hipError_t vc_launch_synth(uint8_t *seq, uint64_t *offs, uint32_t *lens, uint64_t first,
                            uint64_t n_reads, uint32_t L, uint64_t seed, uint64_t thr,
                            const uint8_t *win, const uint8_t *dosage, uint32_t n_snp, hipStream_t st);
+hipError_t vc_launch_unpack(const uint8_t *packed, uint64_t n, uint8_t *out, int n_cu, hipStream_t st);
 hipError_t vc_launch_shard_add(uint32_t *dst, uint32_t *src, uint64_t n, unsigned long long *dst_tally,
                                unsigned long long *src_tally, hipStream_t st);
 #ifdef __cplusplus
diff --git a/kmer-cnt_amd/csrc/vafc_stage.h b/kmer-cnt_amd/csrc/vafc_stage.h
--- a/kmer-cnt_amd/csrc/vafc_stage.h
+++ b/kmer-cnt_amd/csrc/vafc_stage.h
@@ -28,6 +28,8 @@
 	void *map = nullptr;
 	size_t map_len = 0;
 	bool d_one = false;
+	uint8_t *d_pack = nullptr;
+	bool d_pack_own = false;
 };
 
 inline void vc_slot_free(VcSlot &s)
@@ -41,6 +43,7 @@
 		if (s.h_lens) (void)hipHostFree(s.h_lens);
 	}
 	if (s.d_seq) (void)hipFree(s.d_seq);
+	if (s.d_pack_own) (void)hipFree(s.d_pack);
 	if (!s.d_one) {
 		if (s.d_offs) (void)hipFree(s.d_offs);
 		if (s.d_lens) (void)hipFree(s.d_lens);
@@ -72,7 +75,7 @@
 	if (hipHostMalloc((void **)&n.h_seq, bytes, hipHostMallocDefault) != hipSuccess ||
 	    hipHostMalloc((void **)&n.h_offs, reads * sizeof(uint64_t), hipHostMallocDefault) != hipSuccess ||
 	    hipHostMalloc((void **)&n.h_lens, reads * sizeof(uint32_t), hipHostMallocDefault) != hipSuccess ||
-	    hipMalloc((void **)&n.d_seq, bytes) != hipSuccess ||
+	    hipMalloc((void **)&n.d_seq, (bytes + 63) / 64 * 64) != hipSuccess ||
 	    hipMalloc((void **)&n.d_offs, reads * sizeof(uint64_t)) != hipSuccess ||
 	    hipMalloc((void **)&n.d_lens, reads * sizeof(uint32_t)) != hipSuccess) {
 		fprintf(stderr, "[E::vafc] batch buffers of %zu bytes, %zu reads: %s\n", bytes, reads,
@@ -91,6 +94,14 @@
 	n.copied = s.copied;
 	vc_slot_free(s);
 	s = n;
+	return VC_OK;
+}
+
+inline int vc_slot_ensure_pack(VcSlot &s)
+{
+	if (s.d_pack) return VC_OK;
+	HIPCK(hipMalloc((void **)&s.d_pack, s.cap_bytes / 2 + 64));
+	s.d_pack_own = true;
 	return VC_OK;
 }
 
diff --git a/kmer-cnt_amd/csrc/vafc_unpack.hip b/kmer-cnt_amd/csrc/vafc_unpack.hip
--- /dev/null
+++ b/kmer-cnt_amd/csrc/vafc_unpack.hip
@@ -0,0 +1,53 @@
+#include <hip/hip_runtime.h>
+
+#include <stdint.h>
+
+#include "vafc.h"
+#include "vafc_device.h"
+#include "vafc_internal.h"
+
+__device__ __forceinline__ uint32_t vc_nibble_letters(uint32_t c)
+{
+	const uint32_t LET_LO = 0x54474341u;
+	const uint32_t LET_HI = 0x0000554Eu;
+	const uint32_t e = __builtin_amdgcn_perm(LET_HI, LET_LO, c & 0x07070707u);
+	return e | ((c << 2) & (e >> 1) & 0x20202020u);
+}
+
+__global__ void __launch_bounds__(256) vc_unpack_nibbles_kernel(const uint32_t *__restrict__ packed, uint64_t groups,
+                                                               uint2 *__restrict__ out)
+{
+	const uint64_t stride = (uint64_t)gridDim.x * blockDim.x;
+	for (uint64_t g = (uint64_t)blockIdx.x * blockDim.x + threadIdx.x; g < groups; g += stride) {
+		const uint32_t w = packed[g];
+		const uint32_t lo = w & 0x0F0F0F0Fu;
+		const uint32_t hi = (w >> 4) & 0x0F0F0F0Fu;
+		uint2 r;
+		r.x = vc_nibble_letters(__builtin_amdgcn_perm(hi, lo, 0x05010400u));
+		r.y = vc_nibble_letters(__builtin_amdgcn_perm(hi, lo, 0x07030602u));
+		out[g] = r;
+	}
+}
+
+extern "C" hipError_t vc_launch_unpack(const uint8_t *packed, uint64_t n, uint8_t *out, int n_cu, hipStream_t st)
+{
+	const uint64_t groups = (n + 7) / 8;
+	if (!groups) return hipSuccess;
+	uint64_t blocks = (groups + 255) / 256;
+	const uint64_t maxb = (uint64_t)(n_cu > 0 ? n_cu : 256) * 8;
+	if (blocks > maxb) blocks = maxb;
+	hipLaunchKernelGGL(vc_unpack_nibbles_kernel, dim3((unsigned)blocks), dim3(256), 0, st, (const uint32_t *)packed,
+	                   groups, (uint2 *)out);
+	return hipGetLastError();
+}
+
+extern "C" int vc_unpack_device(const void *d_packed, uint64_t n, void *d_out, void *stream)
+{
+	if (!n) return VC_OK;
+	if (!d_packed || !d_out || ((uintptr_t)d_packed & 3) || ((uintptr_t)d_out & 7)) return VC_EINVAL;
+	int dev = 0, n_cu = 0;
+	HIPCK(hipGetDevice(&dev));
+	HIPCK(hipDeviceGetAttribute(&n_cu, hipDeviceAttributeMultiprocessorCount, dev));
+	HIPCK(vc_launch_unpack((const uint8_t *)d_packed, n, (uint8_t *)d_out, n_cu, (hipStream_t)stream));
+	return VC_OK;
+}
diff --git a/kmer-cnt_amd/vafc.py b/kmer-cnt_amd/vafc.py
--- a/kmer-cnt_amd/vafc.py
+++ b/kmer-cnt_amd/vafc.py
@@ -22,6 +22,7 @@
     "vc_table_info", "vc_create_multi", "vc_shard_count", "vc_shard_info", "vc_count_file",
     "vc_count_file_range", "vc_scan_file_range", "vc_ingest_profile", "vc_ingest_profile_ex", "vc_scan_file", "vc_scan_file_parallel",
     "vc_scan_records", "vc_reserve_file_ingest",
+    "vc_ingest_pack_stats", "vc_pack_nibbles", "vc_unpack_nibbles_host", "vc_unpack_device",
     "vc_gz_inflate_parallel", "vc_gz_inflate_zlib", "vc_gz_crc32", "vc_gz_crc32_combine",
     "vc_gz_share_scan", "vc_count_gz_share", "vc_scan_gz_share",
     "vc_gz_share_open", "vc_count_gz_share_held", "vc_scan_gz_share_held", "vc_gz_share_close",
@@ -169,6 +170,10 @@
                                             P, C.c_size_t, P, C.c_size_t]),
         "vc_gz_share_close": (None, [P]),
         "vc_reserve_file_ingest": (C.c_int, [P, C.c_int]),
+        "vc_ingest_pack_stats": (None, [C.POINTER(C.c_uint64), C.POINTER(C.c_uint64)]),
+        "vc_pack_nibbles": (C.c_int64, [P, C.c_size_t, P, C.POINTER(C.c_uint32), C.c_int, C.c_int]),
+        "vc_unpack_nibbles_host": (None, [P, C.c_size_t, P]),
+        "vc_unpack_device": (C.c_int, [P, C.c_uint64, P, P]),
         "vc_fasta_load": (C.c_int, [C.c_char_p, C.POINTER(P)]),
         "vc_fasta_count": (C.c_int, [P]),
         "vc_fasta_name": (C.c_char_p, [P, C.c_int]),
@@ -743,7 +748,34 @@
     for k in ("read_bytes", "copy_bytes", "threads", "copy_mode"):
         d[k] = int(d[k])
     d["pieces"] = int(n)
+    packed, fell = C.c_uint64(0), C.c_uint64(0)
+    lib().vc_ingest_pack_stats(C.byref(packed), C.byref(fell))
+    d["packed_pieces"], d["fallback_pieces"] = int(packed.value), int(fell.value)
     return d
+
+
+PACK_AUTO, PACK_SCALAR, PACK_AVX2 = 0, 1, 2
+
+
+def pack_nibbles(data: bytes, state: int = 0, last: bool = True, impl: int = PACK_AUTO):
+    src = np.frombuffer(bytes(data), np.uint8)
+    dst = np.zeros(len(src) // 2 + 2, np.uint8)
+    st = C.c_uint32(state)
+    n = lib().vc_pack_nibbles(_ptr(src) if len(src) else None, len(src), _ptr(dst), C.byref(st), int(last), impl)
+    if n < 0:
+        return None
+    return dst[:int(n)].tobytes(), int(st.value)
+
+
+def unpack_nibbles_host(packed: bytes, n: int) -> bytes:
+    src = np.frombuffer(bytes(packed) + b"\0", np.uint8)
+    out = np.zeros(max(n, 1), np.uint8)
+    lib().vc_unpack_nibbles_host(_ptr(src), n, _ptr(out))
+    return out[:n].tobytes()
+
+
+def unpack_device(d_packed_ptr, n: int, d_out_ptr, stream=0) -> None:
+    _ck(lib().vc_unpack_device(P(d_packed_ptr), n, P(d_out_ptr), P(stream) if stream else None), "vc_unpack_device")
 
 
 def scan_records(fn: str, cap: int = 1 << 20) -> np.ndarray:
```

After: 36470. 0.91x the previous value.
